# knagrecha/saturn

Hardware: AMD Instinct MI355X
Metric: samples_per_s (higher is better)
Workload: dtype bf16; 1 GPU; model=gptj-6b, global_batch=16, seq_len=512, parallelism=dp1, optimizer=fused_sgd

## Files before the change

### saturn_amd/models/gptj.py

```python

from __future__ import annotations


import os
from dataclasses import dataclass

import torch
import torch.nn as nn

from saturn_amd.ops.functional import (
    fused_gelu,
    FusedLayerNorm,
    apply_rope,
    causal_attention,
    fused_add3,
    fused_cross_entropy,
    rope_tables,
    FusedDropout,
    FusedEmbedding,
    gptj_mlp,
    mlp_fused_supported,
    gptj_branches,
    gptj_branches_supported,
)


@dataclass
class GPTJConfig:
    vocab_size: int = 50400
    n_ctx: int = 512
    n_embd: int = 4096
    n_head: int = 16
    n_layer: int = 28
    rotary_dim: int = 64
    embd_pdrop: float = 0.0
    resid_pdrop: float = 0.0


class GPTJAttention(nn.Module):
    def __init__(self, cfg: GPTJConfig):
        super().__init__()
        self.n_head = cfg.n_head
        self.head_dim = cfg.n_embd // cfg.n_head
        self.rotary_dim = cfg.rotary_dim
        E = cfg.n_embd
        self.q_proj = nn.Linear(E, E, bias=False)
        self.k_proj = nn.Linear(E, E, bias=False)
        self.v_proj = nn.Linear(E, E, bias=False)
        self.out_proj = nn.Linear(E, E, bias=False)
        self.n_ctx = cfg.n_ctx
        self._rope_f32 = rope_tables(cfg.n_ctx, cfg.rotary_dim)

    def _rope(self, device):
        if self._rope_f32[0].device != device:
            self._rope_f32 = tuple(t.to(device) for t in self._rope_f32)
        return self._rope_f32

    def forward(self, x):
        B, T, E = x.shape
        H, D = self.n_head, self.head_dim
        q = self.q_proj(x).view(B, T, H, D)
        k = self.k_proj(x).view(B, T, H, D)
        v = self.v_proj(x).view(B, T, H, D)
        cos, sin = self._rope(x.device)
        q = apply_rope(q, cos, sin)
        k = apply_rope(k, cos, sin)
        q = q.transpose(1, 2)
        k = k.transpose(1, 2)
        v = v.transpose(1, 2)
        o = causal_attention(q, k, v)
        o = o.transpose(1, 2).reshape(B, T, -1)
        return self.out_proj(o)


class GPTJMLP(nn.Module):
    def __init__(self, cfg: GPTJConfig):
        super().__init__()
        E = cfg.n_embd
        self.fc_in = nn.Linear(E, 4 * E)
        self.fc_out = nn.Linear(4 * E, E)

    @staticmethod
    def _plain_linear(m) -> bool:
        return type(m) is nn.Linear and not (
            m._forward_hooks
            or m._forward_pre_hooks
            or m._backward_hooks
            or m._backward_pre_hooks
        )

    def _use_fused(self, x) -> bool:
        if os.environ.get("SAMD_MLP_FUSED", "1") == "0":
            return False
        fi, fo = self.fc_in, self.fc_out
        return (
            x.is_cuda
            and self._plain_linear(fi)
            and self._plain_linear(fo)
            and mlp_fused_supported(x, fi.weight, fi.bias, fo.weight, fo.bias)
        )

    def forward(self, x):
        if self._use_fused(x):
            fi, fo = self.fc_in, self.fc_out
            return gptj_mlp(x, fi.weight, fi.bias, fo.weight, fo.bias)
        return self.fc_out(fused_gelu(self.fc_in(x)))


class GPTJBlock(nn.Module):

    def __init__(self, cfg: GPTJConfig):
        super().__init__()
        self.ln_1 = FusedLayerNorm(cfg.n_embd)
        self.attn = GPTJAttention(cfg)
        self.mlp = GPTJMLP(cfg)
        self.drop = FusedDropout(cfg.resid_pdrop)

    @staticmethod
    def _hooked(m) -> bool:
        return bool(
            m._forward_hooks
            or m._forward_pre_hooks
            or m._backward_hooks
            or m._backward_pre_hooks
        )

    def _use_fused(self, h) -> bool:
        if (os.environ.get("SAMD_MLP_FUSED", "1") == "0"
                or os.environ.get("SAMD_BLOCK_FUSED", "1") == "0"):
            return False
        attn, mlp = self.attn, self.mlp
        if type(attn) is not GPTJAttention or type(mlp) is not GPTJMLP:
            return False
        if not (h.is_cuda and h.dtype == torch.bfloat16 and h.dim() == 3):
            return False
        if self.drop.p != 0.0:
            return False
        from saturn_amd.parallel.sequence import sp_world

        if sp_world() != 1:
            return False
        if any(self._hooked(m) for b in (attn, mlp, self.drop) for m in b.modules()):
            return False
        projs = (attn.q_proj, attn.k_proj, attn.v_proj, attn.out_proj)
        fi, fo = mlp.fc_in, mlp.fc_out
        if not all(GPTJMLP._plain_linear(m) for m in (*projs, fi, fo)):
            return False
        E = h.shape[-1]
        if any(m.bias is not None or m.weight.shape != (E, E)
               or m.weight.dtype != torch.bfloat16 or not m.weight.is_cuda
               for m in projs):
            return False
        return mlp_fused_supported(
            h, fi.weight, fi.bias, fo.weight, fo.bias
        ) and gptj_branches_supported(
            h, attn.n_head, attn.rotary_dim, attn._rope_f32[0].shape[0]
        )

    def forward(self, x):
        h = self.ln_1(x)
        if self._use_fused(h):
            attn, mlp = self.attn, self.mlp
            cos, sin = attn._rope(h.device)
            a, m = gptj_branches(
                h, attn.q_proj.weight, attn.k_proj.weight, attn.v_proj.weight,
                attn.out_proj.weight, mlp.fc_in.weight, mlp.fc_in.bias,
                mlp.fc_out.weight, mlp.fc_out.bias, cos, sin, attn.n_head,
            )
            return fused_add3(x, a, m)
        return fused_add3(x, self.drop(self.attn(h)), self.drop(self.mlp(h)))


class GPTJForCausalLM(nn.Module):
    def __init__(self, cfg: GPTJConfig):
        super().__init__()
        self.cfg = cfg
        self.wte = FusedEmbedding(cfg.vocab_size, cfg.n_embd)
        self.drop = FusedDropout(cfg.embd_pdrop)
        self.h = nn.ModuleList(GPTJBlock(cfg) for _ in range(cfg.n_layer))
        self.ln_f = FusedLayerNorm(cfg.n_embd)
        self.lm_head = nn.Linear(cfg.n_embd, cfg.vocab_size, bias=True)
        self.apply(self._init)

    @staticmethod
    def _init(m):
        if isinstance(m, nn.Linear):
            nn.init.normal_(m.weight, std=0.02)
            if m.bias is not None:
                nn.init.zeros_(m.bias)
        elif isinstance(m, nn.Embedding):
            nn.init.normal_(m.weight, std=0.02)

    def forward(self, input_ids):
        x = self.drop(self.wte(input_ids))
        for block in self.h:
            x = block(x)
        x = self.ln_f(x)
        return self.lm_head(x)


def pretraining_loss(logits, labels):
    return fused_cross_entropy(logits, labels, shift=True)


class _EmbedStage(nn.Module):
    def __init__(self, wte):
        super().__init__()
        self.wte = wte

    def forward(self, input_ids):
        return self.wte(input_ids)


class _HeadStage(nn.Module):
    def __init__(self, ln_f, lm_head):
        super().__init__()
        self.ln_f = ln_f
        self.lm_head = lm_head

    def forward(self, x):
        return self.lm_head(self.ln_f(x))


def as_sequential(model: GPTJForCausalLM) -> nn.Sequential:
    return nn.Sequential(
        _EmbedStage(model.wte), *model.h, _HeadStage(model.ln_f, model.lm_head)
    )


def get_gptj_model(kwargs=None):
    kwargs = kwargs or {}
    cfg = GPTJConfig(
        n_layer=kwargs.get("n_layer", 28),
        n_embd=kwargs.get("n_embd", 4096),
        n_head=kwargs.get("n_head", 16),
        n_ctx=kwargs.get("n_ctx", 512),
        vocab_size=kwargs.get("vocab_size", 50400),
        rotary_dim=kwargs.get("rotary_dim", 64),
        embd_pdrop=kwargs.get("embd_pdrop", 0.0),
        resid_pdrop=kwargs.get("resid_pdrop", 0.0),
    )
    torch.manual_seed(kwargs.get("seed", 0))
    return GPTJForCausalLM(cfg)


class SyntheticTokens(torch.utils.data.Dataset):

    def __init__(self, n: int, seq_len: int, vocab: int, seed: int = 1):
        g = torch.Generator().manual_seed(seed)
        self.data = torch.randint(0, vocab, (n, seq_len), generator=g)

    def __len__(self):
        return len(self.data)

    def __getitem__(self, i):
        return self.data[i]


def _collate(batch):
    x = torch.stack(batch)
    return x, x.clone()


def make_token_dataloader(batch_size=8, seq_len=512, vocab=50400, n_batches=64):
    def get_dataloader():
        return torch.utils.data.DataLoader(
            SyntheticTokens(batch_size * n_batches, seq_len, vocab),
            batch_size=batch_size,
            shuffle=False,
            collate_fn=_collate,
        )

    return get_dataloader
```

### saturn_amd/ops/csrc/bindings.cpp

```cpp

#include <torch/extension.h>
#include <vector>

namespace samd {
void fused_sgd(std::vector<at::Tensor> params, std::vector<at::Tensor> grads,
               std::vector<at::Tensor> moms, std::vector<at::Tensor> masters,
               double lr, double momentum, double weight_decay,
               c10::optional<at::Tensor> grad_scale);
void fused_adam(std::vector<at::Tensor> params, std::vector<at::Tensor> grads,
                std::vector<at::Tensor> ms, std::vector<at::Tensor> vs,
                std::vector<at::Tensor> masters, double lr, double beta1,
                double beta2, double eps, double weight_decay, double bc1,
                double bc2, c10::optional<at::Tensor> grad_scale);
at::Tensor grad_sqsum(std::vector<at::Tensor> tensors, at::Tensor partials);
std::vector<std::pair<int64_t, int64_t>> grad_sqsum_plan(
    std::vector<int64_t> numels);
int64_t grad_sqsum_slots(int64_t n_tensors);
void clip_coef(at::Tensor sq, double max_norm, at::Tensor out);
std::vector<at::Tensor> norm_fwd(at::Tensor x, at::Tensor w,
                                 c10::optional<at::Tensor> b, double eps,
                                 bool rms);
std::vector<at::Tensor> norm_bwd(at::Tensor dy, at::Tensor x, at::Tensor w,
                                 at::Tensor mean, at::Tensor rstd, bool rms,
                                 bool needs_db);
std::vector<at::Tensor> ce_fwd(at::Tensor logits, at::Tensor targets,
                               int64_t Tr, int64_t ignore_index);
at::Tensor ce_bwd(at::Tensor logits, at::Tensor targets, at::Tensor lse,
                  at::Tensor dloss, int64_t Tr, int64_t ignore_index);
void rope_apply(at::Tensor y, at::Tensor x, at::Tensor cos_t, at::Tensor sin_t,
                int64_t t_len, int64_t t_off, bool half_style, bool backward);
at::Tensor gelu_fwd(at::Tensor x);
at::Tensor gelu_bwd(at::Tensor dy, at::Tensor x);
std::vector<at::Tensor> attn_fwd(at::Tensor q, at::Tensor k, at::Tensor v,
                                 bool causal, int64_t kv_len,
                                 c10::optional<at::Tensor> kv_lo);
std::vector<at::Tensor> attn_bwd(at::Tensor dout, at::Tensor q, at::Tensor k,
                                 at::Tensor v, at::Tensor o, at::Tensor lse,
                                 bool causal, int64_t kv_len,
                                 c10::optional<at::Tensor> kv_lo);
std::string attn_dispatch(int64_t T, int64_t D, bool has_lo);
at::Tensor add3(at::Tensor a, at::Tensor b, at::Tensor c);
at::Tensor swiglu_fwd(at::Tensor gate, at::Tensor up);
std::vector<at::Tensor> swiglu_bwd(at::Tensor dout, at::Tensor gate,
                                   at::Tensor up);
at::Tensor embed_fwd(at::Tensor weight, at::Tensor idx);
at::Tensor embed_bwd(at::Tensor dout, at::Tensor idx, long vocab);
at::Tensor dropout_fwd(at::Tensor x, double p, long seed);
at::Tensor dropout_bwd(at::Tensor dout, double p, long seed);
std::vector<at::Tensor> moe_route_fwd(at::Tensor logits, int64_t top_k,
                                      at::ScalarType out_dtype);
at::Tensor moe_route_bwd(at::Tensor logits, at::Tensor ids,
                         at::Tensor dweights);
std::vector<at::Tensor> moe_sort(at::Tensor ids, int64_t n_expert);
at::Tensor moe_permute_fwd(at::Tensor x, at::Tensor order, int64_t top_k);
at::Tensor moe_permute_bwd(at::Tensor dxs, at::Tensor pos);
at::Tensor moe_combine_fwd(at::Tensor y, at::Tensor weights, at::Tensor pos);
std::vector<at::Tensor> moe_combine_bwd(at::Tensor dout, at::Tensor y,
                                        at::Tensor weights, at::Tensor pos);
std::vector<at::Tensor> mlp_act_bwd(at::Tensor d_act, at::Tensor pre,
                                    bool want_dT, bool want_aT);
std::vector<at::Tensor> transpose_colsum(at::Tensor x, bool want_sum);
std::vector<at::Tensor> mlp_bwd(at::Tensor g, at::Tensor h, at::Tensor pre,
                                at::Tensor W_in, at::Tensor W_out,
                                bool use_tn_in, bool use_tn_out);
void transpose_into(at::Tensor x, at::Tensor dst);
at::Tensor rope_bwd_t(at::Tensor dy, at::Tensor cos_t, at::Tensor sin_t,
                      int64_t t_len, int64_t t_off, int64_t dim,
                      at::Tensor dxT);
std::vector<at::Tensor> gptj_branches_bwd(
    at::Tensor g_a, at::Tensor g_m, at::Tensor h, at::Tensor pre, at::Tensor q,
    at::Tensor k, at::Tensor v, at::Tensor o, at::Tensor lse, at::Tensor Wq,
    at::Tensor Wk, at::Tensor Wv, at::Tensor Wo, at::Tensor W_in,
    at::Tensor W_out, at::Tensor cos_t, at::Tensor sin_t, int64_t t_off,
    bool tn_in, bool tn_out, bool tn_qkv, bool tn_o, bool dh_accum);
}

PYBIND11_MODULE(TORCH_EXTENSION_NAME, m) {
  m.doc() = "saturn_amd hand-written CDNA4 (gfx950) kernels";
  m.def("fused_sgd", &samd::fused_sgd, "fused multi-tensor SGD",
        py::arg("params"), py::arg("grads"), py::arg("moms"),
        py::arg("masters"), py::arg("lr"), py::arg("momentum"),
        py::arg("weight_decay"), py::arg("grad_scale") = py::none());
  m.def("fused_adam", &samd::fused_adam, "fused multi-tensor AdamW",
        py::arg("params"), py::arg("grads"), py::arg("ms"), py::arg("vs"),
        py::arg("masters"), py::arg("lr"), py::arg("beta1"),
        py::arg("beta2"), py::arg("eps"), py::arg("weight_decay"),
        py::arg("bc1"), py::arg("bc2"), py::arg("grad_scale") = py::none());
  m.def("grad_sqsum", &samd::grad_sqsum,
        "fp32 sum of squares over a tensor list (no atomics, reproducible)",
        py::arg("tensors"), py::arg("partials"));
  m.def("grad_sqsum_plan", &samd::grad_sqsum_plan,
        "(blocks, threads) of each launch grad_sqsum makes for these sizes",
        py::arg("numels"));
  m.def("grad_sqsum_slots", &samd::grad_sqsum_slots,
        "partials slots a list of n tensors can need (launches x grid cap)",
        py::arg("n_tensors"));
  m.def("clip_coef", &samd::clip_coef,
        "out = {norm, coef, skipped_total} from a squared gradient sum",
        py::arg("sq"), py::arg("max_norm"), py::arg("out"));
  m.def("norm_fwd", &samd::norm_fwd, "LayerNorm/RMSNorm forward");
  m.def("norm_bwd", &samd::norm_bwd, "LayerNorm/RMSNorm backward");
  m.def("ce_fwd", &samd::ce_fwd, "fused cross-entropy forward");
  m.def("ce_bwd", &samd::ce_bwd, "fused cross-entropy backward");
  m.def("rope_apply", &samd::rope_apply,
        "fused rotary embedding (out-of-place, offset table rows)");
  m.def("gelu_fwd", &samd::gelu_fwd, "fused tanh-approx GELU forward");
  m.def("gelu_bwd", &samd::gelu_bwd, "fused tanh-approx GELU backward");
  m.def("attn_fwd", &samd::attn_fwd, "fused flash attention forward",
        py::arg("q"), py::arg("k"), py::arg("v"), py::arg("causal"),
        py::arg("kv_len") = -1, py::arg("kv_lo") = py::none());
  m.def("attn_dispatch", &samd::attn_dispatch,
        "kernel instantiations attn_fwd/attn_bwd launch for (padded T, D)",
        py::arg("T"), py::arg("D"), py::arg("has_lo") = false);
  m.def("attn_bwd", &samd::attn_bwd, "fused flash attention backward",
        py::arg("dout"), py::arg("q"), py::arg("k"), py::arg("v"),
        py::arg("o"), py::arg("lse"), py::arg("causal"),
        py::arg("kv_len") = -1, py::arg("kv_lo") = py::none());
  m.def("add3", &samd::add3, "fused 3-way residual add");
  m.def("swiglu_fwd", &samd::swiglu_fwd, "fused silu(gate)*up");
  m.def("swiglu_bwd", &samd::swiglu_bwd, "fused SwiGLU backward");
  m.def("embed_fwd", &samd::embed_fwd, "token embedding gather");
  m.def("embed_bwd", &samd::embed_bwd, "embedding scatter-add backward");
  m.def("dropout_fwd", &samd::dropout_fwd, "counter-based fused dropout");
  m.def("dropout_bwd", &samd::dropout_bwd, "dropout backward (mask recompute)");
  m.def("moe_route_fwd", &samd::moe_route_fwd,
        "MoE softmax + top-k + renormalise (ties to the lower expert)");
  m.def("moe_route_bwd", &samd::moe_route_bwd, "MoE routing backward");
  m.def("moe_sort", &samd::moe_sort,
        "stable counting sort of (token, slot) pairs by expert");
  m.def("moe_permute_fwd", &samd::moe_permute_fwd,
        "gather token rows into expert order");
  m.def("moe_permute_bwd", &samd::moe_permute_bwd,
        "sum each token's k permuted rows");
  m.def("moe_combine_fwd", &samd::moe_combine_fwd,
        "weighted sum of each token's k expert rows");
  m.def("moe_combine_bwd", &samd::moe_combine_bwd,
        "combine backward: dy and fp32 dweights");
  m.def("mlp_act_bwd", &samd::mlp_act_bwd,
        "GELU backward + transposed d_pre / gelu(pre) + fp32 bias grad",
        py::arg("d_act"), py::arg("pre"), py::arg("want_dT") = true,
        py::arg("want_aT") = true);
  m.def("transpose_colsum", &samd::transpose_colsum,
        "bf16 transpose with optional fp32 column sums");
  m.def("mlp_bwd", &samd::mlp_bwd,
        "GPT-J MLP backward with TN-layout weight gradients");
  m.def("transpose_into", &samd::transpose_into,
        "bf16 transpose stored into a caller-given [N, M] view",
        py::arg("x"), py::arg("dst"));
  m.def("rope_bwd_t", &samd::rope_bwd_t,
        "interleaved RoPE backward that also stores dx^T into a [E, M] view",
        py::arg("dy"), py::arg("cos"), py::arg("sin"), py::arg("t_len"),
        py::arg("t_off"), py::arg("dim"), py::arg("dxT"));
  m.def("gptj_branches_bwd", &samd::gptj_branches_bwd,
        "GPT-J attention + MLP branch backward with shared transposes");
}
```

### saturn_amd/ops/csrc/gptj_block_bwd.hip

```cpp

#include <torch/extension.h>
#include <ATen/hip/HIPContext.h>

#include "common.h"
#include "tile_image.h"

namespace samd {

std::vector<at::Tensor> attn_bwd(at::Tensor dout, at::Tensor q, at::Tensor k,
                                 at::Tensor v, at::Tensor o, at::Tensor lse,
                                 bool causal, int64_t kv_len,
                                 c10::optional<at::Tensor> kv_lo);
std::vector<at::Tensor> mlp_act_bwd(at::Tensor d_act, at::Tensor pre,
                                    bool want_dT, bool want_aT);
void rope_apply(at::Tensor y, at::Tensor x, at::Tensor cos_t, at::Tensor sin_t,
                int64_t t_len, int64_t t_off, bool half_style, bool backward);

namespace {

__global__ void __launch_bounds__(MB_BLOCK)
rope_bwd_t_kernel(const bf16_t* __restrict__ dy, bf16_t* __restrict__ dx,
                  bf16_t* __restrict__ dxT, const float* __restrict__ cos_t,
                  const float* __restrict__ sin_t, long M, long E, int t_len,
                  long t_off, int dim, int half, float sign) {
  __shared__ uint4 img[MB_TILE * 8];

  const int tid = threadIdx.x;
  const int cv = tid & 7;
  const int rp = tid >> 3;
  const int mv = tid & 7;
  const int cr = tid >> 3;
  const long col0 = (long)blockIdx.x * MB_TILE;
  const long col = col0 + cv * 8;
  const bool col_ok = col < E;
  const int j0 = (int)(col % dim);
  const bool rotary = j0 < 2 * half;

  for (int it = 0; it < MB_ROW_ITERS; ++it) {
    const long row0 = ((long)blockIdx.y * MB_ROW_ITERS + it) * MB_TILE;
    if (row0 >= M) break;
    const long row = row0 + 2 * rp;
    const bool ok = col_ok && row < M;

    const short8v zero8 = {0, 0, 0, 0, 0, 0, 0, 0};
    short8v ov[2];
#pragma unroll
    for (int i = 0; i < 2; ++i) {
      ov[i] = zero8;
      if (!ok) continue;
      const short8v xv =
          *reinterpret_cast<const short8v*>(dy + (row + i) * E + col);
      if (rotary) {
        const long trow = (t_off + ((row + i) % t_len)) * (long)half;
#pragma unroll
        for (int e = 0; e < 4; ++e) {
          const int p = j0 / 2 + e;
          const float c = cos_t[trow + p];
          const float s = sin_t[trow + p] * sign;
          bf16_t e0, e1;
          e0.x = (unsigned short)xv[2 * e];
          e1.x = (unsigned short)xv[2 * e + 1];
          const float x0 = toF<bf16_t>(e0);
          const float x1 = toF<bf16_t>(e1);
          ov[i][2 * e] = (short)fromF<bf16_t>(x0 * c - x1 * s).x;
          ov[i][2 * e + 1] = (short)fromF<bf16_t>(x1 * c + x0 * s).x;
        }
      } else {
        ov[i] = xv;
      }
      *reinterpret_cast<short8v*>(dx + (row + i) * E + col) = ov[i];
    }
    unsigned* i32 = reinterpret_cast<unsigned*>(img);
#pragma unroll
    for (int e = 0; e < 8; ++e) {
      i32[img_dword(cv * 8 + e, rp)] =
          (unsigned)(unsigned short)ov[0][e] |
          ((unsigned)(unsigned short)ov[1][e] << 16);
    }
    __syncthreads();

    const long mrow = row0 + mv * 8;
#pragma unroll
    for (int j = 0; j < 2; ++j) {
      const int c = cr + 32 * j;
      if ((col0 + c < E) && (mrow < M))
        *reinterpret_cast<uint4*>(dxT + (col0 + c) * M + mrow) =
            img[img_slot(c, mv)];
    }
    __syncthreads();
  }
}

void check_f32_table(const at::Tensor& t, const char* name) {
  TORCH_CHECK(t.is_cuda() && t.scalar_type() == at::kFloat && t.dim() == 2 &&
                  t.is_contiguous(),
              name, ": expected a contiguous fp32 [T, half] GPU tensor");
}

}

at::Tensor rope_bwd_t(at::Tensor dy, at::Tensor cos_t, at::Tensor sin_t,
                      int64_t t_len, int64_t t_off, int64_t dim,
                      at::Tensor dxT) {
  TORCH_CHECK(dy.is_cuda() && dy.scalar_type() == at::kBFloat16 &&
                  dy.is_contiguous() && dy.numel() > 0,
              "rope_bwd_t dy: expected a contiguous bf16 GPU tensor");
  check_f32_table(cos_t, "rope_bwd_t cos");
  check_f32_table(sin_t, "rope_bwd_t sin");
  const long half = cos_t.size(1);
  TORCH_CHECK(sin_t.sizes() == cos_t.sizes(), "rope_bwd_t: table mismatch");
  TORCH_CHECK(dim > 0 && dim % 8 == 0, "rope_bwd_t: head dim ", dim,
              " must be a positive multiple of 8");
  TORCH_CHECK((2 * half) % 8 == 0 && 2 * half <= dim,
              "rope_bwd_t: rotary dim ", 2 * half,
              " must be a multiple of 8 within the head dim");
  TORCH_CHECK(dy.numel() % dim == 0 && dy.size(-1) == dim,
              "rope_bwd_t: last dim of dy must be the head dim");
  TORCH_CHECK(dy.dim() >= 2, "rope_bwd_t dy: expected [..., heads, dim]");
  const long E = dy.size(-2) * dim;
  const long M = dy.numel() / E;
  TORCH_CHECK(M % 8 == 0, "rope_bwd_t: token count ", M,
              " must be a multiple of 8");
  TORCH_CHECK(t_len > 0 && M % t_len == 0,
              "rope_bwd_t: token count not a multiple of T");
  TORCH_CHECK(t_off >= 0 && cos_t.size(0) >= t_off + t_len,
              "rope_bwd_t: table too short for offset+T");
  TORCH_CHECK(reinterpret_cast<uintptr_t>(dy.data_ptr()) % 16 == 0,
              "rope_bwd_t dy: data must be 16-byte aligned");
  check_operand(dxT, "rope_bwd_t dxT");
  TORCH_CHECK(dxT.size(0) == E && dxT.size(1) == M &&
                  dxT.device() == dy.device(),
              "rope_bwd_t: dxT must be [", E, ", ", M, "], got ", dxT.sizes());

  auto dx = at::empty_like(dy);
  const dim3 grid = tile_grid(M, E);
  auto stream = at::hip::getCurrentHIPStream();
  hipLaunchKernelGGL(rope_bwd_t_kernel, grid, dim3(MB_BLOCK), 0,
                     stream.stream(), bptr(dy), bptr(dx), bptr(dxT),
                     cos_t.data_ptr<float>(), sin_t.data_ptr<float>(), M, E,
                     (int)t_len, (long)t_off, (int)dim, (int)half, -1.f);
  SAMD_CHECK_HIP(hipGetLastError());
  return dx;
}

std::vector<at::Tensor> gptj_branches_bwd(
    at::Tensor g_a, at::Tensor g_m, at::Tensor h, at::Tensor pre, at::Tensor q,
    at::Tensor k, at::Tensor v, at::Tensor o, at::Tensor lse, at::Tensor Wq,
    at::Tensor Wk, at::Tensor Wv, at::Tensor Wo, at::Tensor W_in,
    at::Tensor W_out, at::Tensor cos_t, at::Tensor sin_t, int64_t t_off,
    bool tn_in, bool tn_out, bool tn_qkv, bool tn_o, bool dh_accum) {
  check_operand(g_a, "gptj_branches_bwd g_a");
  check_operand(g_m, "gptj_branches_bwd g_m");
  check_operand(h, "gptj_branches_bwd h");
  check_operand(pre, "gptj_branches_bwd pre");
  check_operand(W_in, "gptj_branches_bwd W_in");
  check_operand(W_out, "gptj_branches_bwd W_out");
  const long M = h.size(0), E = h.size(1), F = pre.size(1);
  TORCH_CHECK(q.dim() == 4 && o.dim() == 4, "gptj_branches_bwd: q, o 4-D");
  const long B = q.size(0), H = q.size(1), T = q.size(2), D = q.size(3);
  TORCH_CHECK(B * T == M && H * D == E && k.sizes() == q.sizes() &&
                  v.sizes() == q.sizes() && o.sizes() == q.sizes(),
              "gptj_branches_bwd: attention shapes do not match h");
  TORCH_CHECK(g_a.sizes() == h.sizes() && g_m.sizes() == h.sizes() &&
                  pre.size(0) == M && W_in.size(0) == F && W_in.size(1) == E &&
                  W_out.size(0) == E && W_out.size(1) == F,
              "gptj_branches_bwd: inconsistent shapes");
  for (const at::Tensor* w : {&Wq, &Wk, &Wv, &Wo}) {
    check_operand(*w, "gptj_branches_bwd projection weight");
    TORCH_CHECK(w->size(0) == E && w->size(1) == E,
                "gptj_branches_bwd: projection weights must be [E, E]");
  }
  auto o_phys = o.permute({0, 2, 1, 3});
  TORCH_CHECK(o_phys.is_contiguous(),
              "gptj_branches_bwd: o must be physically [B,T,H,D]");
  auto o2 = o_phys.view({M, E});
  const bool shared = g_a.data_ptr() == g_m.data_ptr();

  auto gt = transpose_colsum_impl(g_m, true, tn_out || (shared && tn_o));
  at::Tensor gaT;
  if (tn_o) gaT = shared ? gt[0] : transpose_colsum_impl(g_a, false, true)[0];
  at::Tensor hT;
  if (tn_in || tn_qkv) hT = transpose_colsum_impl(h, false, true)[0];

  at::Tensor dh, dW_in, db_in, dW_out;
  {
    at::Tensor d_pre, d_preT, act;
    {
      auto d_act = at::mm(g_m, W_out);
      auto r = mlp_act_bwd(d_act, pre, tn_in, tn_out);
      d_pre = r[0];
      d_preT = r[1];
      act = r[2];
      db_in = r[3];
    }
    dW_out = tn_out ? at::linear(gt[0], act) : at::mm(g_m.t(), act);
    act.reset();
    if (!tn_o) gt[0].reset();
    dW_in = tn_in ? at::linear(d_preT, hT) : at::mm(d_pre.t(), h);
    d_preT.reset();
    if (!tn_qkv) hT.reset();
    dh = at::mm(d_pre, W_in);
  }

  auto d_o = at::mm(g_a, Wo);
  at::Tensor dWo;
  if (tn_o) {
    auto oT = transpose_colsum_impl(o2, false, true)[0];
    dWo = at::linear(gaT, oT);
    gaT.reset();
    gt[0].reset();
  } else {
    dWo = at::mm(g_a.t(), o2);
  }

  at::Tensor dq_r, dk_r, dv;
  {
    auto r = attn_bwd(d_o.view({B, T, H, D}).permute({0, 2, 1, 3}), q, k, v, o,
                      lse, true, T, c10::nullopt);
    dq_r = r[0].permute({0, 2, 1, 3});
    dk_r = r[1].permute({0, 2, 1, 3});
    dv = r[2].permute({0, 2, 1, 3});
    TORCH_CHECK(dq_r.is_contiguous() && dk_r.is_contiguous() &&
                    dv.is_contiguous(),
                "gptj_branches_bwd: attn_bwd layout changed");
  }
  d_o.reset();
  auto dv2 = dv.view({M, E});

  at::Tensor dq, dk, dWq, dWk, dWv;
  if (tn_qkv) {
    auto dqkvT = at::empty({3 * E, M}, h.options());
    dq = rope_bwd_t(dq_r, cos_t, sin_t, T, t_off, D, dqkvT.narrow(0, 0, E));
    dq_r.reset();
    dk = rope_bwd_t(dk_r, cos_t, sin_t, T, t_off, D, dqkvT.narrow(0, E, E));
    dk_r.reset();
    transpose_colsum_impl(dv2, false, true, dqkvT.narrow(0, 2 * E, E));
    auto dW = at::linear(dqkvT, hT);
    dqkvT.reset();
    hT.reset();
    dWq = dW.narrow(0, 0, E);
    dWk = dW.narrow(0, E, E);
    dWv = dW.narrow(0, 2 * E, E);
  } else {
    dq = at::empty_like(dq_r);
    rope_apply(dq, dq_r, cos_t, sin_t, T, t_off, false, true);
    dq_r.reset();
    dk = at::empty_like(dk_r);
    rope_apply(dk, dk_r, cos_t, sin_t, T, t_off, false, true);
    dk_r.reset();
    dWq = at::mm(dq.view({M, E}).t(), h);
    dWk = at::mm(dk.view({M, E}).t(), h);
    dWv = at::mm(dv2.t(), h);
  }

  auto dq2 = dq.view({M, E}), dk2 = dk.view({M, E});
  if (dh_accum) {
    dh.addmm_(dv2, Wv);
    dh.addmm_(dk2, Wk);
    dh.addmm_(dq2, Wq);
  } else {
    dh.add_(at::mm(dv2, Wv));
    dh.add_(at::mm(dk2, Wk));
    dh.add_(at::mm(dq2, Wq));
  }
  return {dh, dWq, dWk, dWv, dWo, dW_in, db_in.to(W_in.scalar_type()),
          dW_out, gt[1].to(W_out.scalar_type())};
}

}
```

### saturn_amd/ops/csrc/layernorm.hip

```cpp

#include <torch/extension.h>
#include <ATen/hip/HIPContext.h>

#include "common.h"

namespace samd {

constexpr int LN_BLOCK = 256;

typedef __attribute__((ext_vector_type(8))) short short8v_ln;

template <typename T>
__device__ __forceinline__ float elemF(const short8v_ln& v, int e) {
  T t;
  t.x = (unsigned short)v[e];
  return toF<T>(t);
}

template <typename T>
__device__ __forceinline__ void setElem(short8v_ln& v, int e, float f) {
  v[e] = (short)fromF<T>(f).x;
}


template <typename T, bool RMS, int GMAX>
__global__ void norm_fwd_vec_kernel(const T* __restrict__ x,
                                    const T* __restrict__ w,
                                    const T* __restrict__ b, T* __restrict__ y,
                                    float* __restrict__ mean_out,
                                    float* __restrict__ rstd_out, int rows,
                                    int cols, float eps) {
  __shared__ float lds[LN_BLOCK / WAVE];
  float cache[8 * GMAX];
  for (int row = blockIdx.x; row < rows; row += gridDim.x) {
    const T* xr = x + (long)row * cols;
    T* yr = y + (long)row * cols;
    float s = 0.f, sq = 0.f;
#pragma unroll
    for (int g = 0; g < GMAX; ++g) {
      const int j = (g * LN_BLOCK + threadIdx.x) * 8;
      if (j < cols) {
        const short8v_ln xv = *reinterpret_cast<const short8v_ln*>(xr + j);
#pragma unroll
        for (int e = 0; e < 8; ++e) {
          const float v = elemF<T>(xv, e);
          cache[g * 8 + e] = v;
          s += v;
          sq += v * v;
        }
      }
    }
    float mean = 0.f;
    if (!RMS) mean = block_sum<LN_BLOCK>(s, lds) / cols;
    const float var = block_sum<LN_BLOCK>(sq, lds) / cols - mean * mean;
    const float rstd = rsqrtf(var + eps);
    if (threadIdx.x == 0) {
      if (!RMS && mean_out) mean_out[row] = mean;
      if (rstd_out) rstd_out[row] = rstd;
    }
#pragma unroll
    for (int g = 0; g < GMAX; ++g) {
      const int j = (g * LN_BLOCK + threadIdx.x) * 8;
      if (j < cols) {
        const short8v_ln wv = *reinterpret_cast<const short8v_ln*>(w + j);
        short8v_ln bv;
        if (!RMS && b) bv = *reinterpret_cast<const short8v_ln*>(b + j);
        short8v_ln ov;
#pragma unroll
        for (int e = 0; e < 8; ++e) {
          const float v = (cache[g * 8 + e] - mean) * rstd;
          float o = v * elemF<T>(wv, e);
          if (!RMS && b) o += elemF<T>(bv, e);
          setElem<T>(ov, e, o);
        }
        *reinterpret_cast<short8v_ln*>(yr + j) = ov;
      }
    }
    __syncthreads();
  }
}

template <typename T, bool RMS>
__global__ void norm_fwd_kernel(const T* __restrict__ x, const T* __restrict__ w,
                                const T* __restrict__ b, T* __restrict__ y,
                                float* __restrict__ mean_out,
                                float* __restrict__ rstd_out, int rows,
                                int cols, float eps) {
  __shared__ float lds[LN_BLOCK / WAVE];
  for (int row = blockIdx.x; row < rows; row += gridDim.x) {
    const T* xr = x + (long)row * cols;
    T* yr = y + (long)row * cols;
    float s = 0.f, sq = 0.f;
    for (int j = threadIdx.x; j < cols; j += LN_BLOCK) {
      float v = (float)xr[j];
      s += v;
      sq += v * v;
    }
    float mean = 0.f;
    if (!RMS) {
      mean = block_sum<LN_BLOCK>(s, lds) / cols;
    }
    float var = block_sum<LN_BLOCK>(sq, lds) / cols - mean * mean;
    float rstd = rsqrtf(var + eps);
    if (threadIdx.x == 0) {
      if (!RMS && mean_out) mean_out[row] = mean;
      if (rstd_out) rstd_out[row] = rstd;
    }
    for (int j = threadIdx.x; j < cols; j += LN_BLOCK) {
      float v = ((float)xr[j] - mean) * rstd;
      float wv = (float)w[j];
      float o = RMS ? v * wv : v * wv + (b ? (float)b[j] : 0.f);
      yr[j] = (T)o;
    }
    __syncthreads();
  }
}


template <typename T, bool RMS, int GMAX>
__global__ void norm_bwd_vec_kernel(const T* __restrict__ dy,
                                    const T* __restrict__ x,
                                    const T* __restrict__ w,
                                    const float* __restrict__ mean,
                                    const float* __restrict__ rstd,
                                    T* __restrict__ dx, float* __restrict__ dw,
                                    float* __restrict__ db, int rows,
                                    int cols) {
  __shared__ float lds[LN_BLOCK / WAVE];
  float dwp[8 * GMAX];
  float dbp[8 * GMAX];
#pragma unroll
  for (int k = 0; k < 8 * GMAX; ++k) { dwp[k] = 0.f; dbp[k] = 0.f; }
  constexpr bool CACHE = GMAX <= 2;
  float c_dyw[CACHE ? 8 * GMAX : 1];
  float c_xh[CACHE ? 8 * GMAX : 1];
  for (int row = blockIdx.x; row < rows; row += gridDim.x) {
    const T* dyr = dy + (long)row * cols;
    const T* xr = x + (long)row * cols;
    T* dxr = dx + (long)row * cols;
    const float mu = RMS ? 0.f : mean[row];
    const float rs = rstd[row];
    float s1 = 0.f, s2 = 0.f;
#pragma unroll
    for (int g = 0; g < GMAX; ++g) {
      const int j = (g * LN_BLOCK + threadIdx.x) * 8;
      if (j < cols) {
        const short8v_ln dyv = *reinterpret_cast<const short8v_ln*>(dyr + j);
        const short8v_ln xv = *reinterpret_cast<const short8v_ln*>(xr + j);
        const short8v_ln wv = *reinterpret_cast<const short8v_ln*>(w + j);
#pragma unroll
        for (int e = 0; e < 8; ++e) {
          const float dyf = elemF<T>(dyv, e);
          const float xh = (elemF<T>(xv, e) - mu) * rs;
          const float dyw = dyf * elemF<T>(wv, e);
          if constexpr (CACHE) {
            c_dyw[g * 8 + e] = dyw;
            c_xh[g * 8 + e] = xh;
          }
          s1 += dyw;
          s2 += dyw * xh;
          dwp[g * 8 + e] += dyf * xh;
          dbp[g * 8 + e] += dyf;
        }
      }
    }
    const float m1 = RMS ? 0.f : block_sum<LN_BLOCK>(s1, lds) / cols;
    const float m2 = block_sum<LN_BLOCK>(s2, lds) / cols;
#pragma unroll
    for (int g = 0; g < GMAX; ++g) {
      const int j = (g * LN_BLOCK + threadIdx.x) * 8;
      if (j < cols) {
        short8v_ln ov;
        if constexpr (CACHE) {
#pragma unroll
          for (int e = 0; e < 8; ++e)
            setElem<T>(ov, e,
                       rs * (c_dyw[g * 8 + e] - m1 - c_xh[g * 8 + e] * m2));
        } else {
          const short8v_ln dyv = *reinterpret_cast<const short8v_ln*>(dyr + j);
          const short8v_ln xv = *reinterpret_cast<const short8v_ln*>(xr + j);
          const short8v_ln wv = *reinterpret_cast<const short8v_ln*>(w + j);
#pragma unroll
          for (int e = 0; e < 8; ++e) {
            const float dyw = elemF<T>(dyv, e) * elemF<T>(wv, e);
            const float xh = (elemF<T>(xv, e) - mu) * rs;
            setElem<T>(ov, e, rs * (dyw - m1 - xh * m2));
          }
        }
        *reinterpret_cast<short8v_ln*>(dxr + j) = ov;
      }
    }
    __syncthreads();
  }
  float* dwr = dw + (long)blockIdx.x * cols;
  float* dbr = db ? db + (long)blockIdx.x * cols : nullptr;
#pragma unroll
  for (int g = 0; g < GMAX; ++g) {
    const int j = (g * LN_BLOCK + threadIdx.x) * 8;
    if (j < cols) {
#pragma unroll
      for (int e = 0; e < 8; ++e) {
        dwr[j + e] = dwp[g * 8 + e];
        if (db) dbr[j + e] = dbp[g * 8 + e];
      }
    }
  }
}


template <typename T, bool RMS, int CPT>
__global__ void norm_bwd_kernel(const T* __restrict__ dy, const T* __restrict__ x,
                                const T* __restrict__ w,
                                const float* __restrict__ mean,
                                const float* __restrict__ rstd,
                                T* __restrict__ dx, float* __restrict__ dw,
                                float* __restrict__ db, int rows, int cols) {
  __shared__ float lds[LN_BLOCK / WAVE];
  float dwp[CPT];
  float dbp[CPT];
#pragma unroll
  for (int k = 0; k < CPT; ++k) { dwp[k] = 0.f; dbp[k] = 0.f; }

  constexpr bool CACHE = (CPT <= 16);
  float c_dyw[CACHE ? CPT : 1];
  float c_xh[CACHE ? CPT : 1];
  for (int row = blockIdx.x; row < rows; row += gridDim.x) {
    const T* dyr = dy + (long)row * cols;
    const T* xr = x + (long)row * cols;
    T* dxr = dx + (long)row * cols;
    const float mu = RMS ? 0.f : mean[row];
    const float rs = rstd[row];
    float s1 = 0.f, s2 = 0.f;
    for (int k = 0, j = threadIdx.x; j < cols; j += LN_BLOCK, ++k) {
      float dyv = (float)dyr[j];
      float xh = ((float)xr[j] - mu) * rs;
      float dyw = dyv * (float)w[j];
      if constexpr (CACHE) {
        c_dyw[k] = dyw;
        c_xh[k] = xh;
      }
      s1 += dyw;
      s2 += dyw * xh;
      dwp[k] += dyv * xh;
      dbp[k] += dyv;
    }
    float m1 = RMS ? 0.f : block_sum<LN_BLOCK>(s1, lds) / cols;
    float m2 = block_sum<LN_BLOCK>(s2, lds) / cols;
    if constexpr (CACHE) {
      for (int k = 0, j = threadIdx.x; j < cols; j += LN_BLOCK, ++k)
        dxr[j] = (T)(rs * (c_dyw[k] - m1 - c_xh[k] * m2));
    } else {
      for (int j = threadIdx.x; j < cols; j += LN_BLOCK) {
        float dyw = (float)dyr[j] * (float)w[j];
        float xh = ((float)xr[j] - mu) * rs;
        dxr[j] = (T)(rs * (dyw - m1 - xh * m2));
      }
    }
    __syncthreads();
  }
  for (int k = 0, j = threadIdx.x; j < cols; j += LN_BLOCK, ++k) {
    atomicAdd(&dw[j], dwp[k]);
    if (db) atomicAdd(&db[j], dbp[k]);
  }
}

static int norm_grid(int rows) { return std::min(rows, 2048); }

std::vector<at::Tensor> norm_fwd(at::Tensor x, at::Tensor w,
                                 c10::optional<at::Tensor> b, double eps,
                                 bool rms) {
  TORCH_CHECK(x.is_cuda() && x.is_contiguous());
  const int cols = (int)x.size(-1);
  const int rows = (int)(x.numel() / cols);
  TORCH_CHECK(cols <= 64 * LN_BLOCK, "row too long for norm kernels");
  auto y = at::empty_like(x);
  auto opts = x.options().dtype(at::kFloat);
  auto mean = rms ? at::Tensor() : at::empty({rows}, opts);
  auto rstd = at::empty({rows}, opts);
  auto stream = at::hip::getCurrentHIPStream();
  dim3 grid(norm_grid(rows)), block(LN_BLOCK);
  const bool vec_ok = x.scalar_type() != at::kFloat && cols % 8 == 0 &&
                      cols <= 8 * LN_BLOCK * 8;

  AT_DISPATCH_FLOATING_TYPES_AND2(
      at::kBFloat16, at::kHalf, x.scalar_type(), "norm_fwd", [&] {
        using T = scalar_t;
        if constexpr (sizeof(T) == 2) {
          if (vec_ok) {
            const int gneeded = (cols + 8 * LN_BLOCK - 1) / (8 * LN_BLOCK);
            void (*kv)(const T*, const T*, const T*, T*, float*, float*, int,
                       int, float);
            if (gneeded <= 2)
              kv = rms ? norm_fwd_vec_kernel<T, true, 2>
                       : norm_fwd_vec_kernel<T, false, 2>;
            else
              kv = rms ? norm_fwd_vec_kernel<T, true, 8>
                       : norm_fwd_vec_kernel<T, false, 8>;
            hipLaunchKernelGGL(kv, grid, block, 0, stream.stream(),
                               reinterpret_cast<const T*>(x.data_ptr()),
                               reinterpret_cast<const T*>(w.data_ptr()),
                               b.has_value()
                                   ? reinterpret_cast<const T*>(b->data_ptr())
                                   : nullptr,
                               reinterpret_cast<T*>(y.data_ptr()),
                               rms ? nullptr : mean.data_ptr<float>(),
                               rstd.data_ptr<float>(), rows, cols,
                               (float)eps);
            return;
          }
        }
        auto k = rms ? norm_fwd_kernel<T, true> : norm_fwd_kernel<T, false>;
        hipLaunchKernelGGL(k, grid, block, 0, stream.stream(),
                           reinterpret_cast<const T*>(x.data_ptr()),
                           reinterpret_cast<const T*>(w.data_ptr()),
                           b.has_value()
                               ? reinterpret_cast<const T*>(b->data_ptr())
                               : nullptr,
                           reinterpret_cast<T*>(y.data_ptr()),
                           rms ? nullptr : mean.data_ptr<float>(),
                           rstd.data_ptr<float>(), rows, cols, (float)eps);
      });
  return {y, mean, rstd};
}

std::vector<at::Tensor> norm_bwd(at::Tensor dy, at::Tensor x, at::Tensor w,
                                 at::Tensor mean, at::Tensor rstd, bool rms,
                                 bool needs_db) {
  TORCH_CHECK(dy.is_cuda() && dy.is_contiguous() && x.is_contiguous());
  const int cols = (int)x.size(-1);
  const int rows = (int)(x.numel() / cols);
  auto dx = at::empty_like(x);
  auto opts = x.options().dtype(at::kFloat);
  auto dw = at::zeros({cols}, opts);
  auto db = needs_db ? at::zeros({cols}, opts) : at::Tensor();
  auto stream = at::hip::getCurrentHIPStream();
  dim3 grid(norm_grid(rows)), block(LN_BLOCK);

  const int cpt_needed = (cols + LN_BLOCK - 1) / LN_BLOCK;
  const bool vec_ok =
      x.scalar_type() != at::kFloat && cols % 8 == 0 && cols <= 8 * LN_BLOCK * 4;
  AT_DISPATCH_FLOATING_TYPES_AND2(
      at::kBFloat16, at::kHalf, x.scalar_type(), "norm_bwd", [&] {
        using T = scalar_t;
        if constexpr (sizeof(T) == 2) {
          if (vec_ok) {
            const int gneeded = (cols + 8 * LN_BLOCK - 1) / (8 * LN_BLOCK);
            void (*kv)(const T*, const T*, const T*, const float*,
                       const float*, T*, float*, float*, int, int);
            if (gneeded <= 2)
              kv = rms ? norm_bwd_vec_kernel<T, true, 2>
                       : norm_bwd_vec_kernel<T, false, 2>;
            else
              kv = rms ? norm_bwd_vec_kernel<T, true, 4>
                       : norm_bwd_vec_kernel<T, false, 4>;
            const int nblk = grid.x;
            auto dw_part = at::empty({nblk, cols}, opts);
            auto db_part =
                needs_db ? at::empty({nblk, cols}, opts) : at::Tensor();
            hipLaunchKernelGGL(kv, grid, block, 0, stream.stream(),
                               reinterpret_cast<const T*>(dy.data_ptr()),
                               reinterpret_cast<const T*>(x.data_ptr()),
                               reinterpret_cast<const T*>(w.data_ptr()),
                               rms ? nullptr : mean.data_ptr<float>(),
                               rstd.data_ptr<float>(),
                               reinterpret_cast<T*>(dx.data_ptr()),
                               dw_part.data_ptr<float>(),
                               needs_db ? db_part.data_ptr<float>() : nullptr,
                               rows, cols);
            at::sum_out(dw, dw_part, {0});
            if (needs_db) at::sum_out(db, db_part, {0});
            return;
          }
        }
        void (*k)(const T*, const T*, const T*, const float*, const float*,
                  T*, float*, float*, int, int);
        if (cpt_needed <= 8)
          k = rms ? norm_bwd_kernel<T, true, 8> : norm_bwd_kernel<T, false, 8>;
        else if (cpt_needed <= 16)
          k = rms ? norm_bwd_kernel<T, true, 16> : norm_bwd_kernel<T, false, 16>;
        else if (cpt_needed <= 32)
          k = rms ? norm_bwd_kernel<T, true, 32> : norm_bwd_kernel<T, false, 32>;
        else
          k = rms ? norm_bwd_kernel<T, true, 64> : norm_bwd_kernel<T, false, 64>;
        hipLaunchKernelGGL(k, grid, block, 0, stream.stream(),
                           reinterpret_cast<const T*>(dy.data_ptr()),
                           reinterpret_cast<const T*>(x.data_ptr()),
                           reinterpret_cast<const T*>(w.data_ptr()),
                           rms ? nullptr : mean.data_ptr<float>(),
                           rstd.data_ptr<float>(),
                           reinterpret_cast<T*>(dx.data_ptr()),
                           dw.data_ptr<float>(),
                           needs_db ? db.data_ptr<float>() : nullptr, rows,
                           cols);
      });
  return {dx, dw, db};
}

}
```

### saturn_amd/ops/csrc/rope.hip

```cpp

#include <torch/extension.h>
#include <ATen/hip/HIPContext.h>

#include "common.h"

namespace samd {

typedef __attribute__((ext_vector_type(8))) short short8v_r;

template <typename T, bool HALF_STYLE>
__global__ void rope_oop_vec_kernel(const T* __restrict__ x, T* __restrict__ y,
                                    const float* __restrict__ cos_t,
                                    const float* __restrict__ sin_t, long n_bt,
                                    int t_len, long t_off, int heads, int dim,
                                    int half, float sign) {
  const int gdim = dim / 8;
  const long total = n_bt * heads * gdim;
  const long stride = (long)gridDim.x * blockDim.x;
  for (long i = blockIdx.x * (long)blockDim.x + threadIdx.x; i < total;
       i += stride) {
    const int gj = (int)(i % gdim);
    const long bth = i / gdim;
    const int h = (int)(bth % heads);
    const long bt = bth / heads;
    const long base = (bt * heads + h) * (long)dim;
    const int j0 = gj * 8;
    const short8v_r xv = *reinterpret_cast<const short8v_r*>(x + base + j0);
    if (j0 >= 2 * half) {
      *reinterpret_cast<short8v_r*>(y + base + j0) = xv;
      continue;
    }
    const long row = (t_off + (bt % t_len)) * (long)half;
    short8v_r ov;
    if constexpr (!HALF_STYLE) {
#pragma unroll
      for (int e = 0; e < 4; ++e) {
        const int p = j0 / 2 + e;
        const float c = cos_t[row + p];
        const float s = sin_t[row + p] * sign;
        T e0, e1;
        e0.x = (unsigned short)xv[2 * e];
        e1.x = (unsigned short)xv[2 * e + 1];
        const float x0 = toF<T>(e0);
        const float x1 = toF<T>(e1);
        ov[2 * e] = (short)fromF<T>(x0 * c - x1 * s).x;
        ov[2 * e + 1] = (short)fromF<T>(x1 * c + x0 * s).x;
      }
    } else {
      const bool low = j0 < half;
      const short8v_r pv = *reinterpret_cast<const short8v_r*>(
          x + base + (low ? j0 + half : j0 - half));
#pragma unroll
      for (int e = 0; e < 8; ++e) {
        const int j = j0 + e;
        const int p = low ? j : j - half;
        const float c = cos_t[row + p];
        const float s = sin_t[row + p] * sign;
        T own, par;
        own.x = (unsigned short)xv[e];
        par.x = (unsigned short)pv[e];
        const float xo = toF<T>(own);
        const float xp = toF<T>(par);
        ov[e] = (short)fromF<T>(low ? xo * c - xp * s : xo * c + xp * s).x;
      }
    }
    *reinterpret_cast<short8v_r*>(y + base + j0) = ov;
  }
}

template <typename T, bool HALF_STYLE>
__global__ void rope_oop_kernel(const T* __restrict__ x, T* __restrict__ y,
                                const float* __restrict__ cos_t,
                                const float* __restrict__ sin_t, long n_bt,
                                int t_len, long t_off, int heads, int dim,
                                int half, float sign) {
  const long total = n_bt * heads * dim;
  const long stride = (long)gridDim.x * blockDim.x;
  for (long i = blockIdx.x * (long)blockDim.x + threadIdx.x; i < total;
       i += stride) {
    const int j = (int)(i % dim);
    const long bth = i / dim;
    const int h = (int)(bth % heads);
    const long bt = bth / heads;
    const long base = (bt * heads + h) * (long)dim;
    if (j >= 2 * half) {
      y[base + j] = x[base + j];
      continue;
    }
    const long row = (t_off + (bt % t_len)) * (long)half;
    int p, jp;
    bool low;
    if (HALF_STYLE) {
      low = j < half;
      p = low ? j : j - half;
      jp = low ? j + half : j - half;
    } else {
      low = (j % 2) == 0;
      p = j / 2;
      jp = low ? j + 1 : j - 1;
    }
    const float c = cos_t[row + p];
    const float s = sin_t[row + p] * sign;
    const float xo = toF<T>(x[base + j]);
    const float xp = toF<T>(x[base + jp]);
    y[base + j] = fromF<T>(low ? xo * c - xp * s : xo * c + xp * s);
  }
}

void rope_apply(at::Tensor y, at::Tensor x, at::Tensor cos_t, at::Tensor sin_t,
                int64_t t_len, int64_t t_off, bool half_style, bool backward) {
  TORCH_CHECK(x.is_cuda() && x.is_contiguous() && y.is_contiguous());
  TORCH_CHECK(y.sizes() == x.sizes() && y.scalar_type() == x.scalar_type());
  const int dim = (int)x.size(-1);
  const int heads = (int)x.size(-2);
  const long n_bt = x.numel() / ((long)dim * heads);
  const int half = (int)cos_t.size(-1);
  TORCH_CHECK(2 * half <= dim, "rotary dim exceeds head dim");
  TORCH_CHECK(n_bt % t_len == 0, "flattened B*T not a multiple of T");
  TORCH_CHECK(cos_t.size(0) >= t_off + t_len && sin_t.size(0) >= t_off + t_len,
              "rope table too short for offset+T");
  TORCH_CHECK(cos_t.scalar_type() == at::kFloat && cos_t.is_contiguous());
  TORCH_CHECK(sin_t.scalar_type() == at::kFloat && sin_t.is_contiguous());
  auto stream = at::hip::getCurrentHIPStream();
  const float sign = backward ? -1.f : 1.f;
  const bool vec_ok = x.scalar_type() != at::kFloat && dim % 8 == 0 &&
                      (half_style ? half % 8 == 0 : (2 * half) % 8 == 0);
  AT_DISPATCH_FLOATING_TYPES_AND2(
      at::kBFloat16, at::kHalf, x.scalar_type(), "rope", [&] {
        const long total =
            vec_ok ? n_bt * heads * (dim / 8) : n_bt * heads * (long)dim;
        const int block = 256;
        dim3 grid((unsigned)std::max<long>(
            1, std::min<long>((total + block - 1) / block, 4096)));
        if (vec_ok) {
          if constexpr (sizeof(scalar_t) == 2) {
            auto k = half_style ? rope_oop_vec_kernel<scalar_t, true>
                                : rope_oop_vec_kernel<scalar_t, false>;
            hipLaunchKernelGGL(
                k, grid, dim3(block), 0, stream.stream(),
                reinterpret_cast<const scalar_t*>(x.data_ptr()),
                reinterpret_cast<scalar_t*>(y.data_ptr()),
                cos_t.data_ptr<float>(), sin_t.data_ptr<float>(), n_bt,
                (int)t_len, (long)t_off, heads, dim, half, sign);
            return;
          }
        }
        auto k = half_style ? rope_oop_kernel<scalar_t, true>
                            : rope_oop_kernel<scalar_t, false>;
        hipLaunchKernelGGL(k, grid, dim3(block), 0, stream.stream(),
                           reinterpret_cast<const scalar_t*>(x.data_ptr()),
                           reinterpret_cast<scalar_t*>(y.data_ptr()),
                           cos_t.data_ptr<float>(), sin_t.data_ptr<float>(),
                           n_bt, (int)t_len, (long)t_off, heads, dim, half,
                           sign);
      });
}

}
```

### saturn_amd/ops/functional.py

```python

from __future__ import annotations

import os
from typing import Tuple

import torch
import torch.nn.functional as F

from saturn_amd.ops import require_ext


class _NormFn(torch.autograd.Function):
    @staticmethod
    def forward(ctx, x, w, b, eps, rms):
        ext = require_ext()
        x = x.contiguous()
        y, mean, rstd = ext.norm_fwd(x, w, b, eps, rms)
        if rms:
            mean = rstd
        ctx.save_for_backward(x, w, mean, rstd)
        ctx.rms = rms
        ctx.has_b = b is not None
        return y

    @staticmethod
    def backward(ctx, dy):
        ext = require_ext()
        x, w, mean, rstd = ctx.saved_tensors
        dx, dw, db = ext.norm_bwd(
            dy.contiguous(), x, w, mean, rstd, ctx.rms, ctx.has_b
        )
        return (
            dx,
            dw.to(w.dtype),
            db.to(w.dtype) if ctx.has_b else None,
            None,
            None,
        )


def fused_layer_norm(x, weight, bias=None, eps: float = 1e-5):
    if x.is_cuda:
        return _NormFn.apply(x, weight, bias, eps, False)
    return F.layer_norm(
        x.float(), (x.shape[-1],),
        weight.float(), bias.float() if bias is not None else None, eps
    ).to(x.dtype)


def fused_rms_norm(x, weight, eps: float = 1e-6):
    if x.is_cuda:
        return _NormFn.apply(x, weight, None, eps, True)
    xf = x.float()
    y = xf * torch.rsqrt(xf.pow(2).mean(-1, keepdim=True) + eps)
    return (y * weight.float()).to(x.dtype)


class FusedLayerNorm(torch.nn.Module):
    def __init__(self, dim: int, eps: float = 1e-5, bias: bool = True):
        super().__init__()
        self.eps = eps
        self.weight = torch.nn.Parameter(torch.ones(dim))
        self.bias = torch.nn.Parameter(torch.zeros(dim)) if bias else None

    def forward(self, x):
        return fused_layer_norm(x, self.weight, self.bias, self.eps)


class FusedRMSNorm(torch.nn.Module):
    def __init__(self, dim: int, eps: float = 1e-6):
        super().__init__()
        self.eps = eps
        self.weight = torch.nn.Parameter(torch.ones(dim))

    def forward(self, x):
        return fused_rms_norm(x, self.weight, self.eps)


class _CeFn(torch.autograd.Function):
    @staticmethod
    def forward(ctx, logits, targets_flat, Tr, ignore_index):
        ext = require_ext()
        loss, lse = ext.ce_fwd(logits, targets_flat, Tr, ignore_index)
        valid = (targets_flat != ignore_index).sum().clamp(min=1)
        ctx.save_for_backward(logits, targets_flat, lse, valid)
        ctx.Tr = Tr
        ctx.ignore_index = ignore_index
        return loss.sum() / valid.float()

    @staticmethod
    def backward(ctx, grad_out):
        ext = require_ext()
        logits, targets_flat, lse, valid = ctx.saved_tensors
        dloss = torch.full_like(lse, 0.0)
        dloss.fill_(1.0)
        dloss = dloss * (grad_out.float() / valid.float())
        dlogits = ext.ce_bwd(
            logits, targets_flat, lse, dloss, ctx.Tr, ctx.ignore_index
        )
        return dlogits, None, None, None


def fused_cross_entropy(
    logits: torch.Tensor,
    targets: torch.Tensor,
    shift: bool = True,
    ignore_index: int = -100,
) -> torch.Tensor:
    B, T, V = logits.shape
    if logits.is_cuda:
        Tr = T - 1 if shift else T
        tg = targets[:, 1:] if shift else targets
        return _CeFn.apply(
            logits.contiguous(), tg.contiguous().view(-1), Tr, ignore_index
        )
    if shift:
        lg = logits[:, :-1].float().reshape(-1, V)
        tg = targets[:, 1:].reshape(-1)
    else:
        lg = logits.float().reshape(-1, V)
        tg = targets.reshape(-1)
    return F.cross_entropy(lg, tg, ignore_index=ignore_index)


def rope_tables(
    T: int,
    rotary_dim: int,
    base: float = 10000.0,
    device=None,
    interleaved: bool = True,
) -> Tuple[torch.Tensor, torch.Tensor]:
    half = rotary_dim // 2
    inv = 1.0 / (base ** (torch.arange(0, half, dtype=torch.float32) * 2 / rotary_dim))
    t = torch.arange(T, dtype=torch.float32)
    freqs = torch.outer(t, inv)
    return freqs.cos().to(device), freqs.sin().to(device)


class _RopeFn(torch.autograd.Function):
    @staticmethod
    def forward(ctx, x, cos_t, sin_t, t_len, t_off, half_style):
        ext = require_ext()
        x = x.contiguous()
        y = torch.empty_like(x)
        ext.rope_apply(y, x, cos_t, sin_t, t_len, t_off, half_style, False)
        ctx.save_for_backward(cos_t, sin_t)
        ctx.meta = (t_len, t_off, half_style)
        return y

    @staticmethod
    def backward(ctx, dy):
        ext = require_ext()
        cos_t, sin_t = ctx.saved_tensors
        t_len, t_off, half_style = ctx.meta
        dy = dy.contiguous()
        dx = torch.empty_like(dy)
        ext.rope_apply(dx, dy, cos_t, sin_t, t_len, t_off, half_style, True)
        return dx, None, None, None, None, None


def _rope_cpu(x, cos_bt, sin_bt, half_style):
    B, T, H, D = x.shape
    half = cos_bt.shape[-1]
    c = cos_bt.view(B, T, 1, half).float()
    s = sin_bt.view(B, T, 1, half).float()
    xf = x.float()
    out = xf.clone()
    if half_style:
        x0 = xf[..., :half]
        x1 = xf[..., half : 2 * half]
        out[..., :half] = x0 * c - x1 * s
        out[..., half : 2 * half] = x1 * c + x0 * s
    else:
        x0 = xf[..., 0 : 2 * half : 2]
        x1 = xf[..., 1 : 2 * half : 2]
        out[..., 0 : 2 * half : 2] = x0 * c - x1 * s
        out[..., 1 : 2 * half : 2] = x1 * c + x0 * s
    return out.to(x.dtype)


def apply_rope(
    x: torch.Tensor,
    cos: torch.Tensor,
    sin: torch.Tensor,
    half_style: bool = False,
) -> torch.Tensor:
    B, T, H, D = x.shape
    half = cos.shape[-1]
    from saturn_amd.parallel.sequence import _STATE as _sp

    off = _sp["rank"] * T if _sp["world"] > 1 else 0
    if cos.shape[0] < off + T:
        raise ValueError(
            "rope table too short for this sequence shard — pass the FULL "
            "table to apply_rope (it slices positions itself)"
        )
    if cos.dtype != torch.float32:
        cos = cos.float()
        sin = sin.float()
    if x.is_cuda:
        return _RopeFn.apply(x, cos.contiguous(), sin.contiguous(), T, off,
                             half_style)
    cos_bt = cos[off : off + T].unsqueeze(0).expand(B, T, half)
    sin_bt = sin[off : off + T].unsqueeze(0).expand(B, T, half)
    return _rope_cpu(x, cos_bt.contiguous(), sin_bt.contiguous(), half_style)


def attention_math(q, k, v, causal: bool = True, kv_lo=None) -> torch.Tensor:
    if kv_lo is not None and not causal:
        raise ValueError("kv_lo needs causal=True")
    scale = 1.0 / (q.shape[-1] ** 0.5)
    s = torch.matmul(q.float(), k.float().transpose(-1, -2)) * scale
    if causal:
        T = q.shape[-2]
        mask = torch.ones(T, T, dtype=torch.bool, device=q.device).tril()
        if kv_lo is not None:
            from saturn_amd.ops.flash import lo_mask

            mask = mask & lo_mask(kv_lo)
        s = s.masked_fill(~mask, float("-inf"))
    p = torch.softmax(s, dim=-1)
    return torch.matmul(p, v.float()).to(q.dtype)


def _attention_core(q, k, v, causal: bool, window=None, kv_lo=None) -> torch.Tensor:
    from saturn_amd.ops import flash

    if q.is_cuda:
        return flash.flash_attention(q, k, v, causal=causal, window=window,
                                     kv_lo=kv_lo)
    if k.shape[1] != q.shape[1]:
        rep = q.shape[1] // k.shape[1]
        k = k.repeat_interleave(rep, dim=1)
        v = v.repeat_interleave(rep, dim=1)
    lo = flash.resolve_lo(q.shape[-2], q.device, causal, window, kv_lo)
    return attention_math(q, k, v, causal=causal, kv_lo=lo)


def _attention(q, k, v, causal: bool, window=None, kv_lo=None) -> torch.Tensor:
    from saturn_amd.parallel.sequence import sp_attention, sp_world

    if sp_world() > 1:
        return sp_attention(
            q, k, v,
            lambda a, b, c: _attention_core(a, b, c, causal, window, kv_lo))
    return _attention_core(q, k, v, causal, window, kv_lo)


def causal_attention(q, k, v, window=None, kv_lo=None) -> torch.Tensor:
    return _attention(q, k, v, causal=True, window=window, kv_lo=kv_lo)


def full_attention(q, k, v) -> torch.Tensor:
    return _attention(q, k, v, causal=False)


class _Add3Fn(torch.autograd.Function):
    @staticmethod
    def forward(ctx, a, b, c):
        ext = require_ext()
        return ext.add3(a.contiguous(), b.contiguous(), c.contiguous())

    @staticmethod
    def backward(ctx, g):
        return g, g, g


def fused_add3(a, b, c):
    if a.is_cuda:
        return _Add3Fn.apply(a, b, c)
    return a + b + c


class _GeluFn(torch.autograd.Function):
    @staticmethod
    def forward(ctx, x):
        ext = require_ext()
        x = x.contiguous()
        ctx.save_for_backward(x)
        return ext.gelu_fwd(x)

    @staticmethod
    def backward(ctx, dy):
        ext = require_ext()
        (x,) = ctx.saved_tensors
        return ext.gelu_bwd(dy.contiguous(), x)


def fused_gelu(x: torch.Tensor) -> torch.Tensor:
    if x.is_cuda and x.dtype in (torch.bfloat16, torch.float16):
        return _GeluFn.apply(x)
    return torch.nn.functional.gelu(x, approximate="tanh")


_MLP_TN_DEFAULT = {"in": True, "out": True}


def _mlp_tn(site: str) -> bool:
    v = os.environ.get("SAMD_MLP_TN_" + site.upper())
    return _MLP_TN_DEFAULT[site] if v is None else v != "0"


def mlp_fused_supported(x, w_in, b_in, w_out, b_out) -> bool:
    if not (x.is_cuda and x.dtype == torch.bfloat16 and x.dim() >= 2):
        return False
    if b_in is None or b_out is None:
        return False
    if any(t.dtype != torch.bfloat16 or not t.is_cuda
           for t in (w_in, b_in, w_out, b_out)):
        return False
    E = x.shape[-1]
    M = x.numel() // E if E else 0
    F_ = w_in.shape[0]
    return (
        M > 0
        and w_in.shape == (F_, E)
        and w_out.shape == (E, F_)
        and M % 8 == 0
        and E % 8 == 0
        and F_ % 8 == 0
    )


class _GPTJMlpFn(torch.autograd.Function):

    @staticmethod
    def forward(ctx, h, w_in, b_in, w_out, b_out):
        ext = require_ext()
        pre = F.linear(h, w_in, b_in).contiguous()
        out = F.linear(ext.gelu_fwd(pre), w_out, b_out)
        ctx.save_for_backward(h, pre, w_in, w_out)
        return out

    @staticmethod
    def backward(ctx, g):
        ext = require_ext()
        h, pre, w_in, w_out = ctx.saved_tensors
        E = h.shape[-1]
        dh, dw_in, db_in, dw_out, db_out = ext.mlp_bwd(
            g.contiguous().view(-1, E),
            h.contiguous().view(-1, E),
            pre.view(-1, pre.shape[-1]),
            w_in.contiguous(),
            w_out.contiguous(),
            _mlp_tn("in"),
            _mlp_tn("out"),
        )
        return dh.view(h.shape), dw_in, db_in, dw_out, db_out


def gptj_mlp(h, w_in, b_in, w_out, b_out):
    return _GPTJMlpFn.apply(h, w_in, b_in, w_out, b_out)


_BLOCK_SITE_DEFAULT = {
    "SAMD_ATTN_TN_QKV": True,
    "SAMD_ATTN_TN_OUT": True,
    "SAMD_DH_ACCUM": False,
}


def _block_site(name: str) -> bool:
    v = os.environ.get(name)
    return _BLOCK_SITE_DEFAULT[name] if v is None else v != "0"


def _same_tensor(a, b) -> bool:
    return (
        a.data_ptr() == b.data_ptr()
        and a.shape == b.shape
        and a.stride() == b.stride()
    )


class _GPTJBranchesFn(torch.autograd.Function):

    @staticmethod
    def forward(ctx, h, wq, wk, wv, wo, w_in, b_in, w_out, b_out, cos, sin,
                n_head, t_off):
        ext = require_ext()
        B, T, E = h.shape
        D = E // n_head
        q = F.linear(h, wq).view(B, T, n_head, D)
        k = F.linear(h, wk).view(B, T, n_head, D)
        v = F.linear(h, wv).view(B, T, n_head, D)
        qr = torch.empty_like(q)
        ext.rope_apply(qr, q, cos, sin, T, t_off, False, False)
        kr = torch.empty_like(k)
        ext.rope_apply(kr, k, cos, sin, T, t_off, False, False)
        del q, k
        qr, kr, v = qr.transpose(1, 2), kr.transpose(1, 2), v.transpose(1, 2)
        o, lse = ext.attn_fwd(qr, kr, v, True, T)
        attn_out = F.linear(o.transpose(1, 2).reshape(B, T, E), wo)
        pre = F.linear(h, w_in, b_in).contiguous()
        mlp_out = F.linear(ext.gelu_fwd(pre), w_out, b_out)
        ctx.save_for_backward(h, pre, qr, kr, v, o, lse, wq, wk, wv, wo,
                              w_in, w_out, cos, sin)
        ctx.t_off = t_off
        return attn_out, mlp_out

    @staticmethod
    def backward(ctx, g_a, g_m):
        ext = require_ext()
        (h, pre, qr, kr, v, o, lse, wq, wk, wv, wo, w_in, w_out, cos,
         sin) = ctx.saved_tensors
        E = h.shape[-1]
        if g_a is None:
            g_a = torch.zeros_like(h)
        if g_m is None:
            g_m = torch.zeros_like(h)
        if _same_tensor(g_a, g_m):
            g_a = g_m = g_m.contiguous().view(-1, E)
        else:
            g_a = g_a.contiguous().view(-1, E)
            g_m = g_m.contiguous().view(-1, E)
        dh, dwq, dwk, dwv, dwo, dw_in, db_in, dw_out, db_out = (
            ext.gptj_branches_bwd(
                g_a, g_m,
                h.contiguous().view(-1, E),
                pre.view(-1, pre.shape[-1]),
                qr, kr, v, o, lse,
                wq.contiguous(), wk.contiguous(), wv.contiguous(),
                wo.contiguous(), w_in.contiguous(), w_out.contiguous(),
                cos, sin, ctx.t_off,
                _mlp_tn("in"), _mlp_tn("out"),
                _block_site("SAMD_ATTN_TN_QKV"),
                _block_site("SAMD_ATTN_TN_OUT"),
                _block_site("SAMD_DH_ACCUM"),
            )
        )
        return (dh.view(h.shape), dwq, dwk, dwv, dwo, dw_in, db_in, dw_out,
                db_out, None, None, None, None)


def gptj_branches_supported(h, n_head, rotary_dim, table_len) -> bool:
    if h.dim() != 3 or n_head <= 0:
        return False
    B, T, E = h.shape
    if E % n_head:
        return False
    D = E // n_head
    return (
        T % 64 == 0
        and T <= table_len
        and D in (64, 128, 256)
        and rotary_dim > 0
        and rotary_dim % 8 == 0
        and rotary_dim <= D
    )


def gptj_branches(h, wq, wk, wv, wo, w_in, b_in, w_out, b_out, cos, sin,
                  n_head):
    return _GPTJBranchesFn.apply(h, wq, wk, wv, wo, w_in, b_in, w_out, b_out,
                                 cos.contiguous(), sin.contiguous(), n_head, 0)


class _SwigluFn(torch.autograd.Function):
    @staticmethod
    def forward(ctx, gate, up):
        ext = require_ext()
        gate = gate.contiguous()
        up = up.contiguous()
        ctx.save_for_backward(gate, up)
        return ext.swiglu_fwd(gate, up)

    @staticmethod
    def backward(ctx, dout):
        ext = require_ext()
        gate, up = ctx.saved_tensors
        dgate, dup = ext.swiglu_bwd(dout.contiguous(), gate, up)
        return dgate, dup


def fused_swiglu(gate, up):
    if gate.is_cuda:
        return _SwigluFn.apply(gate, up)
    return torch.nn.functional.silu(gate) * up


class _EmbedFn(torch.autograd.Function):
    @staticmethod
    def forward(ctx, weight, idx):
        ext = require_ext()
        ctx.save_for_backward(idx)
        ctx.vocab = weight.shape[0]
        return ext.embed_fwd(weight, idx)

    @staticmethod
    def backward(ctx, dout):
        ext = require_ext()
        (idx,) = ctx.saved_tensors
        return ext.embed_bwd(dout, idx, ctx.vocab), None


def fused_embedding(weight, idx):
    if weight.is_cuda:
        return _EmbedFn.apply(weight, idx)
    return F.embedding(idx, weight)


class FusedEmbedding(torch.nn.Embedding):

    def forward(self, idx):
        if (
            self.weight.is_cuda
            and self.padding_idx is None
            and self.max_norm is None
            and not self.sparse
            and self.weight.dtype
            in (torch.bfloat16, torch.float16, torch.float32)
        ):
            return _EmbedFn.apply(self.weight, idx)
        return super().forward(idx)


class _DropoutFn(torch.autograd.Function):
    @staticmethod
    def forward(ctx, x, p, seed):
        ext = require_ext()
        ctx.p = p
        ctx.seed = seed
        return ext.dropout_fwd(x, p, seed)

    @staticmethod
    def backward(ctx, dout):
        ext = require_ext()
        return ext.dropout_bwd(dout.contiguous(), ctx.p, ctx.seed), None, None


def fused_dropout(x, p: float, training: bool = True):
    if p == 0.0 or not training:
        return x
    if x.is_cuda and x.dtype in (torch.bfloat16, torch.float16):
        seed = int(torch.randint(0, 2**62, (1,)).item())
        return _DropoutFn.apply(x.contiguous(), p, seed)
    return F.dropout(x, p, training)


class FusedDropout(torch.nn.Module):
    def __init__(self, p: float = 0.0):
        super().__init__()
        self.p = p

    def forward(self, x):
        return fused_dropout(x, self.p, self.training)

    def extra_repr(self):
        return f"p={self.p}"
```

Before: 63.83 samples/s.

## Fuse ln_1 into GPT-J block autograd with summed-parts norm backward and in-place RoPE

Adds a block-level autograd function that runs ln_1's forward inside the fused branch op and, in backward, feeds the four dh partial products plus the residual gradient straight into a new multi-input layernorm backward kernel. This removes separate dh accumulation passes and the residual add. It also rotates q and k in place with one launch and lets the RoPE backward run in place. In exchange, the residual gradient path now depends on detaching x and requiring both outputs to feed a single add3, which adds brittle coupling and more kernel template variants.

```diff
diff --git a/saturn_amd/models/gptj.py b/saturn_amd/models/gptj.py
--- a/saturn_amd/models/gptj.py
+++ b/saturn_amd/models/gptj.py
@@ -22,6 +22,8 @@
     mlp_fused_supported,
     gptj_branches,
     gptj_branches_supported,
+    gptj_block,
+    gptj_block_tail_enabled,
 )
 
 
@@ -157,7 +159,28 @@
             h, attn.n_head, attn.rotary_dim, attn._rope_f32[0].shape[0]
         )
 
-    def forward(self, x):
+    def _use_tail(self, x) -> bool:
+        ln = self.ln_1
+        if not gptj_block_tail_enabled():
+            return False
+        if type(ln) is not FusedLayerNorm or ln.bias is None:
+            return False
+        if self._hooked(ln):
+            return False
+        return all(p.is_cuda and p.dtype == torch.bfloat16
+                   and p.shape == (x.shape[-1],)
+                   for p in (ln.weight, ln.bias))
+
+    def forward(self, x):
+        if self._use_fused(x) and self._use_tail(x):
+            ln, attn, mlp = self.ln_1, self.attn, self.mlp
+            cos, sin = attn._rope(x.device)
+            return fused_add3(*gptj_block(
+                x, ln.weight, ln.bias, ln.eps,
+                attn.q_proj.weight, attn.k_proj.weight, attn.v_proj.weight,
+                attn.out_proj.weight, mlp.fc_in.weight, mlp.fc_in.bias,
+                mlp.fc_out.weight, mlp.fc_out.bias, cos, sin, attn.n_head,
+            ))
         h = self.ln_1(x)
         if self._use_fused(h):
             attn, mlp = self.attn, self.mlp
diff --git a/saturn_amd/ops/csrc/bindings.cpp b/saturn_amd/ops/csrc/bindings.cpp
--- a/saturn_amd/ops/csrc/bindings.cpp
+++ b/saturn_amd/ops/csrc/bindings.cpp
@@ -23,12 +23,20 @@
 std::vector<at::Tensor> norm_bwd(at::Tensor dy, at::Tensor x, at::Tensor w,
                                  at::Tensor mean, at::Tensor rstd, bool rms,
                                  bool needs_db);
+std::vector<at::Tensor> norm_bwd_sum(std::vector<at::Tensor> parts,
+                                     c10::optional<at::Tensor> resid,
+                                     at::Tensor x, at::Tensor w,
+                                     at::Tensor mean, at::Tensor rstd,
+                                     bool rms, bool needs_db);
 std::vector<at::Tensor> ce_fwd(at::Tensor logits, at::Tensor targets,
                                int64_t Tr, int64_t ignore_index);
 at::Tensor ce_bwd(at::Tensor logits, at::Tensor targets, at::Tensor lse,
                   at::Tensor dloss, int64_t Tr, int64_t ignore_index);
 void rope_apply(at::Tensor y, at::Tensor x, at::Tensor cos_t, at::Tensor sin_t,
                 int64_t t_len, int64_t t_off, bool half_style, bool backward);
+void rope_rotate2_(at::Tensor q, at::Tensor k, at::Tensor cos_t,
+                   at::Tensor sin_t, int64_t t_len, int64_t t_off,
+                   bool half_style);
 at::Tensor gelu_fwd(at::Tensor x);
 at::Tensor gelu_bwd(at::Tensor dy, at::Tensor x);
 std::vector<at::Tensor> attn_fwd(at::Tensor q, at::Tensor k, at::Tensor v,
@@ -66,13 +74,20 @@
 void transpose_into(at::Tensor x, at::Tensor dst);
 at::Tensor rope_bwd_t(at::Tensor dy, at::Tensor cos_t, at::Tensor sin_t,
                       int64_t t_len, int64_t t_off, int64_t dim,
-                      at::Tensor dxT);
+                      at::Tensor dxT, bool inplace);
 std::vector<at::Tensor> gptj_branches_bwd(
     at::Tensor g_a, at::Tensor g_m, at::Tensor h, at::Tensor pre, at::Tensor q,
     at::Tensor k, at::Tensor v, at::Tensor o, at::Tensor lse, at::Tensor Wq,
     at::Tensor Wk, at::Tensor Wv, at::Tensor Wo, at::Tensor W_in,
     at::Tensor W_out, at::Tensor cos_t, at::Tensor sin_t, int64_t t_off,
     bool tn_in, bool tn_out, bool tn_qkv, bool tn_o, bool dh_accum);
+std::vector<at::Tensor> gptj_block_bwd(
+    at::Tensor g, at::Tensor x, at::Tensor ln_w, at::Tensor mean,
+    at::Tensor rstd, at::Tensor h, at::Tensor pre, at::Tensor q, at::Tensor k,
+    at::Tensor v, at::Tensor o, at::Tensor lse, at::Tensor Wq, at::Tensor Wk,
+    at::Tensor Wv, at::Tensor Wo, at::Tensor W_in, at::Tensor W_out,
+    at::Tensor cos_t, at::Tensor sin_t, int64_t t_off, bool tn_in, bool tn_out,
+    bool tn_qkv, bool tn_o, bool dh_accum, bool rope_inplace, bool add_resid);
 }
 
 PYBIND11_MODULE(TORCH_EXTENSION_NAME, m) {
@@ -100,10 +115,20 @@
         py::arg("sq"), py::arg("max_norm"), py::arg("out"));
   m.def("norm_fwd", &samd::norm_fwd, "LayerNorm/RMSNorm forward");
   m.def("norm_bwd", &samd::norm_bwd, "LayerNorm/RMSNorm backward");
+  m.def("norm_bwd_sum", &samd::norm_bwd_sum,
+        "norm backward of the rounded left-to-right sum of 1-4 parts, with "
+        "an optional residual gradient added to dx",
+        py::arg("parts"), py::arg("resid"), py::arg("x"), py::arg("w"),
+        py::arg("mean"), py::arg("rstd"), py::arg("rms"),
+        py::arg("needs_db"));
   m.def("ce_fwd", &samd::ce_fwd, "fused cross-entropy forward");
   m.def("ce_bwd", &samd::ce_bwd, "fused cross-entropy backward");
   m.def("rope_apply", &samd::rope_apply,
         "fused rotary embedding (out-of-place, offset table rows)");
+  m.def("rope_rotate2_", &samd::rope_rotate2_,
+        "interleaved RoPE of q and k in place, rotary slice only, one launch",
+        py::arg("q"), py::arg("k"), py::arg("cos"), py::arg("sin"),
+        py::arg("t_len"), py::arg("t_off"), py::arg("half_style") = false);
   m.def("gelu_fwd", &samd::gelu_fwd, "fused tanh-approx GELU forward");
   m.def("gelu_bwd", &samd::gelu_bwd, "fused tanh-approx GELU backward");
   m.def("attn_fwd", &samd::attn_fwd, "fused flash attention forward",
@@ -150,7 +175,11 @@
   m.def("rope_bwd_t", &samd::rope_bwd_t,
         "interleaved RoPE backward that also stores dx^T into a [E, M] view",
         py::arg("dy"), py::arg("cos"), py::arg("sin"), py::arg("t_len"),
-        py::arg("t_off"), py::arg("dim"), py::arg("dxT"));
+        py::arg("t_off"), py::arg("dim"), py::arg("dxT"),
+        py::arg("inplace") = false);
   m.def("gptj_branches_bwd", &samd::gptj_branches_bwd,
         "GPT-J attention + MLP branch backward with shared transposes");
+  m.def("gptj_block_bwd", &samd::gptj_block_bwd,
+        "GPT-J block backward: branches, then ln_1's backward summing the "
+        "four terms of dh and the residual gradient in one pass");
 }
diff --git a/saturn_amd/ops/csrc/gptj_block_bwd.hip b/saturn_amd/ops/csrc/gptj_block_bwd.hip
--- a/saturn_amd/ops/csrc/gptj_block_bwd.hip
+++ b/saturn_amd/ops/csrc/gptj_block_bwd.hip
@@ -13,11 +13,17 @@
                                  c10::optional<at::Tensor> kv_lo);
 std::vector<at::Tensor> mlp_act_bwd(at::Tensor d_act, at::Tensor pre,
                                     bool want_dT, bool want_aT);
+std::vector<at::Tensor> norm_bwd_sum(std::vector<at::Tensor> parts,
+                                     c10::optional<at::Tensor> resid,
+                                     at::Tensor x, at::Tensor w,
+                                     at::Tensor mean, at::Tensor rstd,
+                                     bool rms, bool needs_db);
 void rope_apply(at::Tensor y, at::Tensor x, at::Tensor cos_t, at::Tensor sin_t,
                 int64_t t_len, int64_t t_off, bool half_style, bool backward);
 
 namespace {
 
+template <bool INPLACE>
 __global__ void __launch_bounds__(MB_BLOCK)
 rope_bwd_t_kernel(const bf16_t* __restrict__ dy, bf16_t* __restrict__ dx,
                   bf16_t* __restrict__ dxT, const float* __restrict__ cos_t,
@@ -48,8 +54,8 @@
     for (int i = 0; i < 2; ++i) {
       ov[i] = zero8;
       if (!ok) continue;
-      const short8v xv =
-          *reinterpret_cast<const short8v*>(dy + (row + i) * E + col);
+      const short8v xv = *reinterpret_cast<const short8v*>(
+          (INPLACE ? dx : dy) + (row + i) * E + col);
       if (rotary) {
         const long trow = (t_off + ((row + i) % t_len)) * (long)half;
 #pragma unroll
@@ -68,7 +74,8 @@
       } else {
         ov[i] = xv;
       }
-      *reinterpret_cast<short8v*>(dx + (row + i) * E + col) = ov[i];
+      if (!INPLACE || rotary)
+        *reinterpret_cast<short8v*>(dx + (row + i) * E + col) = ov[i];
     }
     unsigned* i32 = reinterpret_cast<unsigned*>(img);
 #pragma unroll
@@ -101,7 +108,7 @@
 
 at::Tensor rope_bwd_t(at::Tensor dy, at::Tensor cos_t, at::Tensor sin_t,
                       int64_t t_len, int64_t t_off, int64_t dim,
-                      at::Tensor dxT) {
+                      at::Tensor dxT, bool inplace) {
   TORCH_CHECK(dy.is_cuda() && dy.scalar_type() == at::kBFloat16 &&
                   dy.is_contiguous() && dy.numel() > 0,
               "rope_bwd_t dy: expected a contiguous bf16 GPU tensor");
@@ -132,23 +139,31 @@
                   dxT.device() == dy.device(),
               "rope_bwd_t: dxT must be [", E, ", ", M, "], got ", dxT.sizes());
 
-  auto dx = at::empty_like(dy);
+  auto dx = inplace ? dy : at::empty_like(dy);
   const dim3 grid = tile_grid(M, E);
   auto stream = at::hip::getCurrentHIPStream();
-  hipLaunchKernelGGL(rope_bwd_t_kernel, grid, dim3(MB_BLOCK), 0,
-                     stream.stream(), bptr(dy), bptr(dx), bptr(dxT),
-                     cos_t.data_ptr<float>(), sin_t.data_ptr<float>(), M, E,
-                     (int)t_len, (long)t_off, (int)dim, (int)half, -1.f);
+  if (inplace)
+    hipLaunchKernelGGL(rope_bwd_t_kernel<true>, grid, dim3(MB_BLOCK), 0,
+                       stream.stream(), static_cast<const bf16_t*>(nullptr),
+                       bptr(dx), bptr(dxT),
+                       cos_t.data_ptr<float>(), sin_t.data_ptr<float>(), M, E,
+                       (int)t_len, (long)t_off, (int)dim, (int)half, -1.f);
+  else
+    hipLaunchKernelGGL(rope_bwd_t_kernel<false>, grid, dim3(MB_BLOCK), 0,
+                       stream.stream(), bptr(dy), bptr(dx), bptr(dxT),
+                       cos_t.data_ptr<float>(), sin_t.data_ptr<float>(), M, E,
+                       (int)t_len, (long)t_off, (int)dim, (int)half, -1.f);
   SAMD_CHECK_HIP(hipGetLastError());
   return dx;
 }
 
-std::vector<at::Tensor> gptj_branches_bwd(
+static std::vector<at::Tensor> branches_bwd_impl(
     at::Tensor g_a, at::Tensor g_m, at::Tensor h, at::Tensor pre, at::Tensor q,
     at::Tensor k, at::Tensor v, at::Tensor o, at::Tensor lse, at::Tensor Wq,
     at::Tensor Wk, at::Tensor Wv, at::Tensor Wo, at::Tensor W_in,
     at::Tensor W_out, at::Tensor cos_t, at::Tensor sin_t, int64_t t_off,
-    bool tn_in, bool tn_out, bool tn_qkv, bool tn_o, bool dh_accum) {
+    bool tn_in, bool tn_out, bool tn_qkv, bool tn_o, bool dh_accum,
+    bool rope_inplace, std::vector<at::Tensor>* dh_parts) {
   check_operand(g_a, "gptj_branches_bwd g_a");
   check_operand(g_m, "gptj_branches_bwd g_m");
   check_operand(h, "gptj_branches_bwd h");
@@ -230,9 +245,11 @@
   at::Tensor dq, dk, dWq, dWk, dWv;
   if (tn_qkv) {
     auto dqkvT = at::empty({3 * E, M}, h.options());
-    dq = rope_bwd_t(dq_r, cos_t, sin_t, T, t_off, D, dqkvT.narrow(0, 0, E));
+    dq = rope_bwd_t(dq_r, cos_t, sin_t, T, t_off, D, dqkvT.narrow(0, 0, E),
+                    rope_inplace);
     dq_r.reset();
-    dk = rope_bwd_t(dk_r, cos_t, sin_t, T, t_off, D, dqkvT.narrow(0, E, E));
+    dk = rope_bwd_t(dk_r, cos_t, sin_t, T, t_off, D, dqkvT.narrow(0, E, E),
+                    rope_inplace);
     dk_r.reset();
     transpose_colsum_impl(dv2, false, true, dqkvT.narrow(0, 2 * E, E));
     auto dW = at::linear(dqkvT, hT);
@@ -258,13 +275,50 @@
     dh.addmm_(dv2, Wv);
     dh.addmm_(dk2, Wk);
     dh.addmm_(dq2, Wq);
+    if (dh_parts) *dh_parts = {dh};
+  } else if (dh_parts) {
+    *dh_parts = {dh, at::mm(dv2, Wv), at::mm(dk2, Wk), at::mm(dq2, Wq)};
   } else {
     dh.add_(at::mm(dv2, Wv));
     dh.add_(at::mm(dk2, Wk));
     dh.add_(at::mm(dq2, Wq));
   }
+  if (dh_parts) dh.reset();
   return {dh, dWq, dWk, dWv, dWo, dW_in, db_in.to(W_in.scalar_type()),
           dW_out, gt[1].to(W_out.scalar_type())};
 }
 
-}
+std::vector<at::Tensor> gptj_branches_bwd(
+    at::Tensor g_a, at::Tensor g_m, at::Tensor h, at::Tensor pre, at::Tensor q,
+    at::Tensor k, at::Tensor v, at::Tensor o, at::Tensor lse, at::Tensor Wq,
+    at::Tensor Wk, at::Tensor Wv, at::Tensor Wo, at::Tensor W_in,
+    at::Tensor W_out, at::Tensor cos_t, at::Tensor sin_t, int64_t t_off,
+    bool tn_in, bool tn_out, bool tn_qkv, bool tn_o, bool dh_accum) {
+  return branches_bwd_impl(g_a, g_m, h, pre, q, k, v, o, lse, Wq, Wk, Wv, Wo,
+                           W_in, W_out, cos_t, sin_t, t_off, tn_in, tn_out,
+                           tn_qkv, tn_o, dh_accum, false, nullptr);
+}
+
+std::vector<at::Tensor> gptj_block_bwd(
+    at::Tensor g, at::Tensor x, at::Tensor ln_w, at::Tensor mean,
+    at::Tensor rstd, at::Tensor h, at::Tensor pre, at::Tensor q, at::Tensor k,
+    at::Tensor v, at::Tensor o, at::Tensor lse, at::Tensor Wq, at::Tensor Wk,
+    at::Tensor Wv, at::Tensor Wo, at::Tensor W_in, at::Tensor W_out,
+    at::Tensor cos_t, at::Tensor sin_t, int64_t t_off, bool tn_in, bool tn_out,
+    bool tn_qkv, bool tn_o, bool dh_accum, bool rope_inplace,
+    bool add_resid) {
+  check_operand(x, "gptj_block_bwd x");
+  TORCH_CHECK(x.sizes() == h.sizes(), "gptj_block_bwd: x and h differ");
+  std::vector<at::Tensor> parts;
+  auto r = branches_bwd_impl(g, g, h, pre, q, k, v, o, lse, Wq, Wk, Wv, Wo,
+                             W_in, W_out, cos_t, sin_t, t_off, tn_in, tn_out,
+                             tn_qkv, tn_o, dh_accum, rope_inplace && tn_qkv,
+                             &parts);
+  auto n = norm_bwd_sum(parts, add_resid ? c10::make_optional(g) : c10::nullopt,
+                        x, ln_w, mean, rstd, false, true);
+  parts.clear();
+  return {n[0], n[1].to(ln_w.scalar_type()), n[2].to(ln_w.scalar_type()),
+          r[1], r[2], r[3], r[4], r[5], r[6], r[7], r[8]};
+}
+
+}
diff --git a/saturn_amd/ops/csrc/layernorm.hip b/saturn_amd/ops/csrc/layernorm.hip
--- a/saturn_amd/ops/csrc/layernorm.hip
+++ b/saturn_amd/ops/csrc/layernorm.hip
@@ -117,8 +117,32 @@
 }
 
 
-template <typename T, bool RMS, int GMAX>
-__global__ void norm_bwd_vec_kernel(const T* __restrict__ dy,
+template <typename T, int NP>
+struct NormParts {
+  const T* p[NP];
+};
+
+template <typename T, int NP>
+__device__ __forceinline__ void load_parts(const NormParts<T, NP>& parts,
+                                           long off, short8v_ln (&pv)[NP]) {
+#pragma unroll
+  for (int k = 0; k < NP; ++k)
+    pv[k] = *reinterpret_cast<const short8v_ln*>(parts.p[k] + off);
+}
+
+template <typename T, int NP>
+__device__ __forceinline__ float chain_sum(const short8v_ln (&pv)[NP], int e) {
+  float v = elemF<T>(pv[0], e);
+#pragma unroll
+  for (int k = 1; k < NP; ++k) v = toF<T>(fromF<T>(v + elemF<T>(pv[k], e)));
+  return v;
+}
+
+template <typename T, bool RMS, int GMAX, int NP, bool RESID>
+__global__ void __launch_bounds__(
+    (GMAX > 2 && (NP > 1 || RESID)) ? LN_BLOCK : 1024)
+norm_bwd_vec_kernel(const NormParts<T, NP> parts,
+                                    const T* __restrict__ resid,
                                     const T* __restrict__ x,
                                     const T* __restrict__ w,
                                     const float* __restrict__ mean,
@@ -135,9 +159,9 @@
   float c_dyw[CACHE ? 8 * GMAX : 1];
   float c_xh[CACHE ? 8 * GMAX : 1];
   for (int row = blockIdx.x; row < rows; row += gridDim.x) {
-    const T* dyr = dy + (long)row * cols;
-    const T* xr = x + (long)row * cols;
-    T* dxr = dx + (long)row * cols;
+    const long roff = (long)row * cols;
+    const T* xr = x + roff;
+    T* dxr = dx + roff;
     const float mu = RMS ? 0.f : mean[row];
     const float rs = rstd[row];
     float s1 = 0.f, s2 = 0.f;
@@ -145,12 +169,13 @@
     for (int g = 0; g < GMAX; ++g) {
       const int j = (g * LN_BLOCK + threadIdx.x) * 8;
       if (j < cols) {
-        const short8v_ln dyv = *reinterpret_cast<const short8v_ln*>(dyr + j);
+        short8v_ln pv[NP];
+        load_parts<T, NP>(parts, roff + j, pv);
         const short8v_ln xv = *reinterpret_cast<const short8v_ln*>(xr + j);
         const short8v_ln wv = *reinterpret_cast<const short8v_ln*>(w + j);
 #pragma unroll
         for (int e = 0; e < 8; ++e) {
-          const float dyf = elemF<T>(dyv, e);
+          const float dyf = chain_sum<T, NP>(pv, e);
           const float xh = (elemF<T>(xv, e) - mu) * rs;
           const float dyw = dyf * elemF<T>(wv, e);
           if constexpr (CACHE) {
@@ -177,15 +202,23 @@
             setElem<T>(ov, e,
                        rs * (c_dyw[g * 8 + e] - m1 - c_xh[g * 8 + e] * m2));
         } else {
-          const short8v_ln dyv = *reinterpret_cast<const short8v_ln*>(dyr + j);
+          short8v_ln pv[NP];
+          load_parts<T, NP>(parts, roff + j, pv);
           const short8v_ln xv = *reinterpret_cast<const short8v_ln*>(xr + j);
           const short8v_ln wv = *reinterpret_cast<const short8v_ln*>(w + j);
 #pragma unroll
           for (int e = 0; e < 8; ++e) {
-            const float dyw = elemF<T>(dyv, e) * elemF<T>(wv, e);
+            const float dyw = chain_sum<T, NP>(pv, e) * elemF<T>(wv, e);
             const float xh = (elemF<T>(xv, e) - mu) * rs;
             setElem<T>(ov, e, rs * (dyw - m1 - xh * m2));
           }
+        }
+        if constexpr (RESID) {
+          const short8v_ln rv =
+              *reinterpret_cast<const short8v_ln*>(resid + roff + j);
+#pragma unroll
+          for (int e = 0; e < 8; ++e)
+            setElem<T>(ov, e, elemF<T>(ov, e) + elemF<T>(rv, e));
         }
         *reinterpret_cast<short8v_ln*>(dxr + j) = ov;
       }
@@ -323,6 +356,42 @@
   return {y, mean, rstd};
 }
 
+template <typename T, int NP, bool RESID>
+static void norm_bwd_vec_launch(const at::Tensor* parts,
+                                const at::Tensor* resid, const at::Tensor& x,
+                                const at::Tensor& w, const at::Tensor& mean,
+                                const at::Tensor& rstd, at::Tensor& dx,
+                                at::Tensor& dw, at::Tensor& db, bool rms,
+                                bool needs_db, int rows, int cols) {
+  const int gneeded = (cols + 8 * LN_BLOCK - 1) / (8 * LN_BLOCK);
+  void (*kv)(const NormParts<T, NP>, const T*, const T*, const T*,
+             const float*, const float*, T*, float*, float*, int, int);
+  if (gneeded <= 2)
+    kv = rms ? norm_bwd_vec_kernel<T, true, 2, NP, RESID>
+             : norm_bwd_vec_kernel<T, false, 2, NP, RESID>;
+  else
+    kv = rms ? norm_bwd_vec_kernel<T, true, 4, NP, RESID>
+             : norm_bwd_vec_kernel<T, false, 4, NP, RESID>;
+  NormParts<T, NP> pp;
+  for (int k = 0; k < NP; ++k)
+    pp.p[k] = reinterpret_cast<const T*>(parts[k].data_ptr());
+  const int nblk = norm_grid(rows);
+  auto opts = x.options().dtype(at::kFloat);
+  auto dw_part = at::empty({nblk, cols}, opts);
+  auto db_part = needs_db ? at::empty({nblk, cols}, opts) : at::Tensor();
+  auto stream = at::hip::getCurrentHIPStream();
+  hipLaunchKernelGGL(
+      kv, dim3(nblk), dim3(LN_BLOCK), 0, stream.stream(), pp,
+      RESID ? reinterpret_cast<const T*>(resid->data_ptr()) : nullptr,
+      reinterpret_cast<const T*>(x.data_ptr()),
+      reinterpret_cast<const T*>(w.data_ptr()),
+      rms ? nullptr : mean.data_ptr<float>(), rstd.data_ptr<float>(),
+      reinterpret_cast<T*>(dx.data_ptr()), dw_part.data_ptr<float>(),
+      needs_db ? db_part.data_ptr<float>() : nullptr, rows, cols);
+  at::sum_out(dw, dw_part, {0});
+  if (needs_db) at::sum_out(db, db_part, {0});
+}
+
 std::vector<at::Tensor> norm_bwd(at::Tensor dy, at::Tensor x, at::Tensor w,
                                  at::Tensor mean, at::Tensor rstd, bool rms,
                                  bool needs_db) {
@@ -344,31 +413,9 @@
         using T = scalar_t;
         if constexpr (sizeof(T) == 2) {
           if (vec_ok) {
-            const int gneeded = (cols + 8 * LN_BLOCK - 1) / (8 * LN_BLOCK);
-            void (*kv)(const T*, const T*, const T*, const float*,
-                       const float*, T*, float*, float*, int, int);
-            if (gneeded <= 2)
-              kv = rms ? norm_bwd_vec_kernel<T, true, 2>
-                       : norm_bwd_vec_kernel<T, false, 2>;
-            else
-              kv = rms ? norm_bwd_vec_kernel<T, true, 4>
-                       : norm_bwd_vec_kernel<T, false, 4>;
-            const int nblk = grid.x;
-            auto dw_part = at::empty({nblk, cols}, opts);
-            auto db_part =
-                needs_db ? at::empty({nblk, cols}, opts) : at::Tensor();
-            hipLaunchKernelGGL(kv, grid, block, 0, stream.stream(),
-                               reinterpret_cast<const T*>(dy.data_ptr()),
-                               reinterpret_cast<const T*>(x.data_ptr()),
-                               reinterpret_cast<const T*>(w.data_ptr()),
-                               rms ? nullptr : mean.data_ptr<float>(),
-                               rstd.data_ptr<float>(),
-                               reinterpret_cast<T*>(dx.data_ptr()),
-                               dw_part.data_ptr<float>(),
-                               needs_db ? db_part.data_ptr<float>() : nullptr,
-                               rows, cols);
-            at::sum_out(dw, dw_part, {0});
-            if (needs_db) at::sum_out(db, db_part, {0});
+            norm_bwd_vec_launch<T, 1, false>(&dy, nullptr, x, w, mean, rstd,
+                                             dx, dw, db, rms, needs_db, rows,
+                                             cols);
             return;
           }
         }
@@ -396,4 +443,76 @@
   return {dx, dw, db};
 }
 
-}
+std::vector<at::Tensor> norm_bwd_sum(std::vector<at::Tensor> parts,
+                                     c10::optional<at::Tensor> resid,
+                                     at::Tensor x, at::Tensor w,
+                                     at::Tensor mean, at::Tensor rstd,
+                                     bool rms, bool needs_db) {
+  const int np = (int)parts.size();
+  TORCH_CHECK(np >= 1 && np <= 4, "norm_bwd_sum: expected 1-4 parts, got ", np);
+  TORCH_CHECK(x.is_cuda() && x.is_contiguous() && x.dim() >= 1 &&
+                  x.numel() > 0,
+              "norm_bwd_sum x: expected a contiguous GPU tensor");
+  const bool has_resid = resid.has_value() && resid->defined();
+  auto aligned = [](const at::Tensor& t) {
+    return reinterpret_cast<uintptr_t>(t.data_ptr()) % 16 == 0;
+  };
+  bool all_aligned = aligned(x) && aligned(w);
+  auto check_like_x = [&](const at::Tensor& t, const char* name) {
+    TORCH_CHECK(t.is_cuda() && t.device() == x.device() &&
+                    t.scalar_type() == x.scalar_type() && t.is_contiguous() &&
+                    t.numel() == x.numel() && t.size(-1) == x.size(-1),
+                "norm_bwd_sum ", name,
+                ": expected a contiguous tensor with x's shape and dtype");
+    all_aligned = all_aligned && aligned(t);
+  };
+  for (const auto& p : parts) check_like_x(p, "part");
+  if (has_resid) check_like_x(*resid, "resid");
+  const long cols_l = x.size(-1);
+  TORCH_CHECK(w.is_cuda() && w.is_contiguous() && w.numel() == cols_l &&
+                  w.scalar_type() == x.scalar_type(),
+              "norm_bwd_sum w: expected [cols] of x's dtype");
+  const long rows_l = x.numel() / cols_l;
+  TORCH_CHECK(rstd.numel() == rows_l && (rms || mean.numel() == rows_l),
+              "norm_bwd_sum: mean/rstd must hold one value per row");
+
+  const bool vec_ok = x.scalar_type() == at::kBFloat16 && cols_l % 8 == 0 &&
+                      cols_l <= 8 * LN_BLOCK * 4 && all_aligned;
+  if (!vec_ok) {
+    at::Tensor dy = parts[0];
+    for (int k = 1; k < np; ++k) dy = at::add(dy, parts[k]);
+    auto r = norm_bwd(dy, x, w, mean, rstd, rms, needs_db);
+    if (has_resid) r[0] = at::add(*resid, r[0]);
+    return r;
+  }
+
+  using T = c10::BFloat16;
+  const int cols = (int)cols_l, rows = (int)rows_l;
+  auto dx = at::empty_like(x);
+  auto opts = x.options().dtype(at::kFloat);
+  auto dw = at::zeros({cols}, opts);
+  auto db = needs_db ? at::zeros({cols}, opts) : at::Tensor();
+  const at::Tensor* rp = has_resid ? &*resid : nullptr;
+#define SAMD_NORM_SUM(NP)                                                    \
+  case NP:                                                                   \
+    if (has_resid)                                                           \
+      norm_bwd_vec_launch<T, NP, true>(parts.data(), rp, x, w, mean, rstd,   \
+                                       dx, dw, db, rms, needs_db, rows,      \
+                                       cols);                                \
+    else                                                                     \
+      norm_bwd_vec_launch<T, NP, false>(parts.data(), rp, x, w, mean, rstd,  \
+                                        dx, dw, db, rms, needs_db, rows,     \
+                                        cols);                               \
+    break;
+  switch (np) {
+    SAMD_NORM_SUM(1)
+    SAMD_NORM_SUM(2)
+    SAMD_NORM_SUM(3)
+    SAMD_NORM_SUM(4)
+  }
+#undef SAMD_NORM_SUM
+  SAMD_CHECK_HIP(hipGetLastError());
+  return {dx, dw, db};
+}
+
+}
diff --git a/saturn_amd/ops/csrc/rope.hip b/saturn_amd/ops/csrc/rope.hip
--- a/saturn_amd/ops/csrc/rope.hip
+++ b/saturn_amd/ops/csrc/rope.hip
@@ -105,6 +105,91 @@
     const float xp = toF<T>(x[base + jp]);
     y[base + j] = fromF<T>(low ? xo * c - xp * s : xo * c + xp * s);
   }
+}
+
+template <typename T>
+__global__ void rope_rotate2_kernel(T* xa, T* xb,
+                                    const float* __restrict__ cos_t,
+                                    const float* __restrict__ sin_t, long n_bt,
+                                    int t_len, long t_off, int heads, int dim,
+                                    int half, float sign) {
+  T* x = blockIdx.y ? xb : xa;
+  const int grot = 2 * half / 8;
+  const long total = n_bt * heads * grot;
+  const long stride = (long)gridDim.x * blockDim.x;
+  for (long i = blockIdx.x * (long)blockDim.x + threadIdx.x; i < total;
+       i += stride) {
+    const int gj = (int)(i % grot);
+    const long bth = i / grot;
+    const long bt = bth / heads;
+    const long base = bth * (long)dim;
+    const int j0 = gj * 8;
+    const short8v_r xv = *reinterpret_cast<const short8v_r*>(x + base + j0);
+    const long row = (t_off + (bt % t_len)) * (long)half;
+    short8v_r ov;
+#pragma unroll
+    for (int e = 0; e < 4; ++e) {
+      const int p = j0 / 2 + e;
+      const float c = cos_t[row + p];
+      const float s = sin_t[row + p] * sign;
+      T e0, e1;
+      e0.x = (unsigned short)xv[2 * e];
+      e1.x = (unsigned short)xv[2 * e + 1];
+      const float x0 = toF<T>(e0);
+      const float x1 = toF<T>(e1);
+      ov[2 * e] = (short)fromF<T>(x0 * c - x1 * s).x;
+      ov[2 * e + 1] = (short)fromF<T>(x1 * c + x0 * s).x;
+    }
+    *reinterpret_cast<short8v_r*>(x + base + j0) = ov;
+  }
+}
+
+void rope_rotate2_(at::Tensor q, at::Tensor k, at::Tensor cos_t,
+                   at::Tensor sin_t, int64_t t_len, int64_t t_off,
+                   bool half_style) {
+  TORCH_CHECK(!half_style,
+              "rope_rotate2_: half-split pairs span two vectors and cannot "
+              "be rotated in place; use rope_apply");
+  for (const at::Tensor* t : {&q, &k}) {
+    TORCH_CHECK(t->is_cuda() && t->scalar_type() == at::kBFloat16 &&
+                    t->is_contiguous() && t->dim() >= 2 && t->numel() > 0,
+                "rope_rotate2_: expected contiguous bf16 GPU tensors "
+                "[..., heads, dim]");
+    TORCH_CHECK(reinterpret_cast<uintptr_t>(t->data_ptr()) % 16 == 0,
+                "rope_rotate2_: data must be 16-byte aligned");
+  }
+  TORCH_CHECK(k.sizes() == q.sizes() && k.device() == q.device(),
+              "rope_rotate2_: q and k must have one shape and device");
+  TORCH_CHECK(cos_t.is_cuda() && cos_t.scalar_type() == at::kFloat &&
+                  cos_t.dim() == 2 && cos_t.is_contiguous() &&
+                  sin_t.is_cuda() && sin_t.scalar_type() == at::kFloat &&
+                  sin_t.is_contiguous() && sin_t.sizes() == cos_t.sizes(),
+              "rope_rotate2_: tables must be contiguous fp32 [T, half]");
+  const int dim = (int)q.size(-1);
+  const int heads = (int)q.size(-2);
+  const long n_bt = q.numel() / ((long)dim * heads);
+  const int half = (int)cos_t.size(1);
+  TORCH_CHECK(dim % 8 == 0 && half > 0 && (2 * half) % 8 == 0 &&
+                  2 * half <= dim,
+              "rope_rotate2_: head dim ", dim, " and rotary dim ", 2 * half,
+              " must be multiples of 8, rotary within the head");
+  TORCH_CHECK(t_len > 0 && n_bt % t_len == 0,
+              "rope_rotate2_: flattened B*T not a multiple of T");
+  TORCH_CHECK(t_off >= 0 && cos_t.size(0) >= t_off + t_len,
+              "rope_rotate2_: table too short for offset+T");
+  using T = c10::BFloat16;
+  const long total = n_bt * heads * (2 * half / 8);
+  const int block = 256;
+  dim3 grid((unsigned)std::max<long>(
+                1, std::min<long>((total + block - 1) / block, 4096)),
+            2);
+  auto stream = at::hip::getCurrentHIPStream();
+  hipLaunchKernelGGL(rope_rotate2_kernel<T>, grid, dim3(block), 0,
+                     stream.stream(), reinterpret_cast<T*>(q.data_ptr()),
+                     reinterpret_cast<T*>(k.data_ptr()),
+                     cos_t.data_ptr<float>(), sin_t.data_ptr<float>(), n_bt,
+                     (int)t_len, (long)t_off, heads, dim, half, 1.f);
+  SAMD_CHECK_HIP(hipGetLastError());
 }
 
 void rope_apply(at::Tensor y, at::Tensor x, at::Tensor cos_t, at::Tensor sin_t,
diff --git a/saturn_amd/ops/functional.py b/saturn_amd/ops/functional.py
--- a/saturn_amd/ops/functional.py
+++ b/saturn_amd/ops/functional.py
@@ -456,6 +456,87 @@
                                  cos.contiguous(), sin.contiguous(), n_head, 0)
 
 
+_BLOCK_SITE_DEFAULT.update({
+    "SAMD_BLOCK_TAIL": True,
+    "SAMD_ROPE_INPLACE": True,
+})
+
+
+def gptj_block_tail_enabled() -> bool:
+    return _block_site("SAMD_BLOCK_TAIL")
+
+
+class _GPTJBranchesFnLN(torch.autograd.Function):
+
+    @staticmethod
+    def forward(ctx, x, ln_w, ln_b, eps, wq, wk, wv, wo, w_in, b_in, w_out,
+                b_out, cos, sin, n_head, t_off):
+        ext = require_ext()
+        B, T, E = x.shape
+        D = E // n_head
+        x = x.contiguous()
+        h, mean, rstd = ext.norm_fwd(x, ln_w, ln_b, eps, False)
+        q = F.linear(h, wq).view(B, T, n_head, D)
+        k = F.linear(h, wk).view(B, T, n_head, D)
+        v = F.linear(h, wv).view(B, T, n_head, D)
+        if _block_site("SAMD_ROPE_INPLACE"):
+            ext.rope_rotate2_(q, k, cos, sin, T, t_off)
+            qr, kr = q, k
+        else:
+            qr = torch.empty_like(q)
+            ext.rope_apply(qr, q, cos, sin, T, t_off, False, False)
+            kr = torch.empty_like(k)
+            ext.rope_apply(kr, k, cos, sin, T, t_off, False, False)
+        del q, k
+        qr, kr, v = qr.transpose(1, 2), kr.transpose(1, 2), v.transpose(1, 2)
+        o, lse = ext.attn_fwd(qr, kr, v, True, T)
+        attn_out = F.linear(o.transpose(1, 2).reshape(B, T, E), wo)
+        pre = F.linear(h, w_in, b_in).contiguous()
+        mlp_out = F.linear(ext.gelu_fwd(pre), w_out, b_out)
+        ctx.save_for_backward(x, mean, rstd, h, pre, qr, kr, v, o, lse, ln_w,
+                              wq, wk, wv, wo, w_in, w_out, cos, sin)
+        ctx.t_off = t_off
+        return attn_out, mlp_out
+
+    @staticmethod
+    def backward(ctx, g_a, g_m):
+        ext = require_ext()
+        (x, mean, rstd, h, pre, qr, kr, v, o, lse, ln_w, wq, wk, wv, wo,
+         w_in, w_out, cos, sin) = ctx.saved_tensors
+        E = x.shape[-1]
+        if g_a is None or g_m is None or not _same_tensor(g_a, g_m):
+            raise RuntimeError(
+                "_GPTJBranchesFnLN: both outputs must feed one add3 with "
+                "x.detach() (gptj_block); use gptj_branches otherwise")
+        g = g_m.contiguous().view(-1, E)
+        (dx, dln_w, dln_b, dwq, dwk, dwv, dwo, dw_in, db_in, dw_out,
+         db_out) = ext.gptj_block_bwd(
+            g, x.view(-1, E), ln_w, mean, rstd,
+            h.view(-1, E), pre.view(-1, pre.shape[-1]),
+            qr, kr, v, o, lse,
+            wq.contiguous(), wk.contiguous(), wv.contiguous(),
+            wo.contiguous(), w_in.contiguous(), w_out.contiguous(),
+            cos, sin, ctx.t_off,
+            _mlp_tn("in"), _mlp_tn("out"),
+            _block_site("SAMD_ATTN_TN_QKV"),
+            _block_site("SAMD_ATTN_TN_OUT"),
+            _block_site("SAMD_DH_ACCUM"),
+            _block_site("SAMD_ROPE_INPLACE"),
+            ctx.needs_input_grad[0],
+        )
+        return (dx.view(x.shape) if ctx.needs_input_grad[0] else None,
+                dln_w, dln_b, None, dwq, dwk, dwv, dwo, dw_in, db_in, dw_out,
+                db_out, None, None, None, None)
+
+
+def gptj_block(x, ln_w, ln_b, eps, wq, wk, wv, wo, w_in, b_in, w_out, b_out,
+               cos, sin, n_head):
+    a, m = _GPTJBranchesFnLN.apply(
+        x, ln_w, ln_b, eps, wq, wk, wv, wo, w_in, b_in, w_out, b_out,
+        cos.contiguous(), sin.contiguous(), n_head, 0)
+    return x.detach(), a, m
+
+
 class _SwigluFn(torch.autograd.Function):
     @staticmethod
     def forward(ctx, gate, up):
```

Result: no change. 64.39 samples/s, median of 6 (+0.9%).
